# heng-hw/SpaCap3D

Measured on AMD Instinct MI355X. Metric: scenes/sec (40k pts, 256 proposals) fwd+bwd, higher is better.
Workload: dtype f32; 1 GPU; cfg2: synthetic ScanRefer-shaped scans, 40000 pts x (xyz+1 ch), 256 proposals, 8 scenes/GPU; full training step (SpaCapNet fwd + loss + bwd + grad all-reduce + Adam); global_batch=8, parallelism=dp1, hip_graph=True, fps_prefetch_side_stream=True, prefetch_as_graph=True, reserved_cus_forward=8, geometry_prefetch=True, deferred_weight_gradients=True, params=9290918, allreduce_bytes=35572416

## Files before the change

include/spacap_hip.h:

```cpp
#ifndef SPACAP_HIP_H
#define SPACAP_HIP_H

#include <stddef.h>
#include <stdint.h>

#ifdef __cplusplus
extern "C" {
#endif

#define SPACAP_ABI_VERSION 5

#define SPACAP_OK 0
#define SPACAP_E_INVALID (-1)
#define SPACAP_E_LAUNCH (-2)
#define SPACAP_E_NO_DEVICE (-3)

typedef void *spacap_stream_t;

int spacap_abi_version(void);
const char *spacap_last_error(void);
int spacap_device_count(void);

int spacap_opt_n_threads(int work_size);


size_t spacap_fps_workspace_bytes(int B, int N);
int spacap_fps_f32(const float *xyz, int B, int N, int m, void *workspace, int32_t *idx,
                   spacap_stream_t stream);

int spacap_gather_points_f32(const float *points, const int32_t *idx, int B, int C, int N, int m,
                             float *out, spacap_stream_t stream);
int spacap_gather_points_grad_f32(const float *grad_out, const int32_t *idx, int B, int C, int N,
                                  int m, float *grad_points, spacap_stream_t stream);


int spacap_ball_query_f32(const float *new_xyz, const float *xyz, int B, int N, int m,
                          float radius, int nsample, int32_t *idx, spacap_stream_t stream);

size_t spacap_ball_query_grid_workspace_bytes(int B, int N);
int spacap_ball_query_grid_f32(const float *new_xyz, const float *xyz, int B, int N, int m, float radius, int nsample,
                               int32_t *idx, void *workspace, size_t workspace_bytes, spacap_stream_t stream);


int spacap_group_points_f32(const float *points, const int32_t *idx, int B, int C, int N, int P,
                            int S, float *out, spacap_stream_t stream);
size_t spacap_group_points_grad_workspace_bytes(int B, int C, int N, int P, int S);
int spacap_group_points_grad_f32(const float *grad_out, const int32_t *idx, int B, int C, int N,
                                 int P, int S, float *grad_points, void *workspace,
                                 spacap_stream_t stream);


int spacap_group_max_f32(const float *x, long rows, int S, float *out, uint8_t *arg,
                         spacap_stream_t stream);
int spacap_group_max_grad_f32(const float *grad_out, const uint8_t *arg, long rows, int S,
                              float *grad_in, spacap_stream_t stream);


int spacap_three_nn_f32(const float *unknown, const float *known, int B, int n, int m,
                        float *dist2, int32_t *idx, spacap_stream_t stream);
int spacap_three_nn_weights_f32(const float *unknown, const float *known, int B, int n, int m,
                                float *weight, int32_t *idx, spacap_stream_t stream);
int spacap_gather_xyz_f32(const float *xyz, const int32_t *idx, int B, int N, int m, float *out, spacap_stream_t stream);
int spacap_three_interpolate_f32(const float *points, const int32_t *idx, const float *weight,
                                 int B, int C, int m, int n, float *out, spacap_stream_t stream);
int spacap_three_interpolate_grad_f32(const float *grad_out, const int32_t *idx,
                                      const float *weight, int B, int C, int n, int m,
                                      float *grad_points, spacap_stream_t stream);
int spacap_three_interpolate_grad_pm_f32(const float *grad_pm, const int32_t *idx, const float *weight, int B, int C,
                                         int n, int m, float *grad_points_pm, spacap_stream_t stream);
int spacap_fp_concat_fwd_f32(const float *known, int known_pm, const int32_t *idx, const float *weight, const float *skip, int B,
                             int K1, int K2, int m, int n, float *out, spacap_stream_t stream);
int spacap_fp_concat_bwd_f32(const float *g, int B, int K1, int K2, int n, float *g1, float *g2, spacap_stream_t stream);


int spacap_mha_fwd_f32(const float *q, const float *k, const float *v, long q_sb, long q_sh,
                       long q_sl, long k_sb, long k_sh, long k_sl, long v_sb, long v_sh, long v_sl,
                       const uint8_t *mask, long mask_sb, long mask_sq, const float *bias,
                       long bias_sb, long bias_sh, long bias_sq, int B, int h, int Lq, int Lk,
                       int d_k, float scale, float dropout_p, uint64_t seed, const uint64_t *seed_dev,
                       float *out, float *p_out, float *stats, spacap_stream_t stream);

size_t spacap_mha_bwd_workspace_bytes(int B, int h, int Lq);
int spacap_mha_bwd_f32(const float *q, const float *k, const float *v, long q_sb, long q_sh,
                       long q_sl, long k_sb, long k_sh, long k_sl, long v_sb, long v_sh, long v_sl,
                       const uint8_t *mask, long mask_sb, long mask_sq, const float *bias,
                       long bias_sb, long bias_sh, long bias_sq, int B, int h, int Lq, int Lk,
                       int d_k, float scale, float dropout_p, uint64_t seed, const uint64_t *seed_dev,
                       const float *stats, const float *d_out, const float *d_p, void *workspace,
                       float *dq, float *dk, float *dv, long grad_row_stride, spacap_stream_t stream);

int spacap_mha_bwd_delta_f32(const float *q, const float *k, const float *v, long q_sb, long q_sh,
                             long q_sl, long k_sb, long k_sh, long k_sl, long v_sb, long v_sh, long v_sl,
                             const uint8_t *mask, long mask_sb, long mask_sq, const float *bias,
                             long bias_sb, long bias_sh, long bias_sq, int B, int h, int Lq, int Lk,
                             int d_k, float scale, float dropout_p, uint64_t seed, const uint64_t *seed_dev,
                             const float *stats, const float *d_out, const float *delta,
                             float *dq, float *dk, float *dv, long grad_row_stride, spacap_stream_t stream);

size_t spacap_bn_workspace_bytes(int C);
int spacap_bn_set_single_launch(int enabled);
int spacap_bn_stats_f32(const float *z, int B, int C, long L, float eps, float momentum, float *running_mean,
                        float *running_var, float *stats, void *workspace, spacap_stream_t stream);
int spacap_bn_relu_train_f32(const float *z, int B, int C, long L, float eps, float momentum, float *running_mean,
                             float *running_var, const float *gamma, const float *beta, float *stats, float *out,
                             void *workspace, spacap_stream_t stream);
int spacap_bn_relu_apply_f32(const float *z, const float *stats, const float *gamma, const float *beta, int B,
                             int C, long L, float *out, spacap_stream_t stream);
int spacap_bn_relu_max_f32(const float *z, const float *stats, const float *gamma, const float *beta, int B, int C,
                           int P, int S, float *out, uint8_t *arg, spacap_stream_t stream);
int spacap_bn_relu_bwd_f32(const float *z, const float *stats, const float *gamma, const float *beta,
                           const float *dA, int B, int C, long L, float *dz, float *dgamma, float *dbeta,
                           void *workspace, spacap_stream_t stream);
int spacap_bn_relu_max_bwd_f32(const float *z, const float *stats, const float *gamma, const float *beta,
                               const float *dP, const uint8_t *arg, int B, int C, int P, int S, float *dz,
                               float *dgamma, float *dbeta, void *workspace, spacap_stream_t stream);

int spacap_relation_feature_fwd_f32(const float *P, const float *V, long v_sb, long v_sh, long v_sl, int B,
                                    int H, int K, int D, float *R, spacap_stream_t stream);
int spacap_relation_feature_bwd_f32(const float *dR, const float *P, const float *V, long v_sb, long v_sh,
                                    long v_sl, int B, int H, int K, int D, float *dP, float *dV,
                                    spacap_stream_t stream);

int spacap_relation_l1_fwd_f32(const float *P, const float *U, const float *b1, int B, int H, int K, int C,
                               float *H1, spacap_stream_t stream);
int spacap_relation_l1_isplit(void);
int spacap_relation_l1_supported(int H, int K, int C);
int spacap_relation_l1_blocks(int B, int K, int C);
int spacap_relation_l1_bwd_f32(const float *dH1, const float *H1, const float *P, const float *U, int B, int H,
                               int K, int C, float *dP, float *dU, float *db_part, spacap_stream_t stream);

int spacap_relation_fused_leave_cus(int n);
int spacap_relation_fused_supported(int H, int K, int C, int n_out);
int spacap_relation_fused_nparts(int B, int K);
int spacap_relation_fused_zsplit(int B, int K, int nparts);
int spacap_relation_fused_part_floats(void);
int spacap_relation_fused_fwd_f32(const float *P, const float *U, const float *b1, const float *W2, const float *b2,
                                  const float *W3, const float *b3, int B, int K, float *hid2, float *pred,
                                  spacap_stream_t stream);
int spacap_relation_fused_bwd_f32(const float *dpred, const float *hid2, const float *P, const float *U, const float *b1,
                                  const float *W2, const float *W3, int B, int K, int nparts, int zslots, float *dP,
                                  float *dU, float *part, spacap_stream_t stream);
int spacap_relation_fused_sel_zsplit(int B, int K, int nparts);
size_t spacap_relation_fused_sel_workspace_bytes(int B, int K);
int spacap_relation_fused_sel_lists_f32(const float *dpred, int B, int K, int zslots, float *dP, float *dU, void *workspace,
                                        spacap_stream_t stream);
int spacap_relation_fused_bwd_sel_f32(const float *dpred, const float *hid2, const float *P, const float *U, const float *b1,
                                      const float *W2, const float *W3, int B, int K, int nparts, int zslots, float *dP,
                                      float *dU, float *part, void *workspace, spacap_stream_t stream);

int spacap_caption_prep_fwd_f32(const float *xyz, const float *ref, const float *src, const float *memory,
                                const int64_t *tok, const float *emb, const float *pe, int B, int K, int D, int T, int V,
                                float p, uint64_t seed, const uint64_t *seed_dev, float *x0, uint8_t *mask, int64_t *idx,
                                float *dist, uint8_t *good, float *pred, int32_t *counter, spacap_stream_t stream);
int spacap_caption_prep_bwd_f32(const float *g, const int64_t *tok, const int64_t *idx, int B, int K, int D, int T, int V,
                                float p, uint64_t seed, const uint64_t *seed_dev, float *d_rows, float *d_emb,
                                spacap_stream_t stream);
int spacap_caption_prep_rows_fwd_f32(const float *src, const float *memory, const int64_t *prop, const int64_t *tok,
                                     const float *emb, const float *pe, int B, int K, int M, int S, int D, int T, int V, float p,
                                     uint64_t seed, const uint64_t *seed_dev, float *x0, uint8_t *mask, spacap_stream_t stream);
int spacap_caption_prep_rows_bwd_f32(const float *g, const int64_t *tok, const int64_t *prop, int B, int K, int M, int S, int D,
                                     int T, int V, float p, uint64_t seed, const uint64_t *seed_dev, float *d_rows, float *d_emb,
                                     spacap_stream_t stream);


int spacap_layernorm_fwd_f32(const float *x, const float *a, const float *b, long rows, int D, float eps,
                             float *y, float *stats, spacap_stream_t stream);
size_t spacap_layernorm_bwd_workspace_bytes(long rows, int D);
int spacap_layernorm_bwd_f32(const float *x, const float *a, const float *stats, const float *dy, long rows,
                             int D, float eps, float *dx, float *da, float *db, void *workspace,
                             spacap_stream_t stream);
int spacap_layernorm_bwd_add_f32(const float *x, const float *a, const float *stats, const float *dy, const float *addend,
                                 long rows, int D, float eps, float *dx, float *da, float *db, void *workspace,
                                 spacap_stream_t stream);

int spacap_sa_nparts(void);
int spacap_sa_wgrad_slabs(long R, int CK, int CP, int pooled);
int spacap_sa_mlp_supported(int C1, int C2, int C3);
int spacap_sa_l1_fwd_f32(const float *Y, const float *feat, const float *xyz, const float *new_xyz,
                         const int32_t *idx, const float *W1, int ldw, float rdiv, int B, int Np, int N, int S,
                         int C1, float *z1, double *part, spacap_stream_t stream);
int spacap_sa_bn_finalize_f32(const double *part, int C, long count, float eps, float momentum, const float *gamma,
                              const float *beta, float *running_mean, float *running_var, float *stats,
                              spacap_stream_t stream);
int spacap_sa_mid_fwd_f32(const float *zin, const float *st_in, const float *W, long R, int Cin, int Cout,
                          float *zout, double *part, spacap_stream_t stream);
int spacap_gemm_rows_supported(int Cin, int Cout);
int spacap_gemm_rows_f32(const float *x, const float *W, long R, int Cin, int Cout, float *out, spacap_stream_t stream);
int spacap_sa_mid_fwd_pool_supported(int Cin, int Cout, int S);
int spacap_sa_reserve_cus(int n);
int spacap_sa_mid_fwd_pool_f32(const float *zin, const float *st_in, const float *W, const float *gamma_out, long R,
                               int Cin, int Cout, int S, float *zout, double *part, float *cand_v, uint8_t *cand_i,
                               spacap_stream_t stream);
int spacap_sa_pool_finalize_f32(const float *cand_v, const uint8_t *cand_i, const float *stats, const float *gamma, long G,
                                int S, int C, float *out, uint8_t *arg, float *zmax, spacap_stream_t stream);
int spacap_sa_pool_fwd_f32(const float *z, const float *stats, long G, int S, int C, float *out, uint8_t *arg,
                           spacap_stream_t stream);
int spacap_sa_pool_bwd_f32(const float *dout, const float *out, const uint8_t *arg, const float *z, const float *zmax,
                           const float *stats, long G, int S, int C, float *dym, double *part,
                           spacap_stream_t stream);
long spacap_sa_l3bwd_part_floats(int C2, int C3);
int spacap_sa_l3bwd_dw_f32(const float *partW, int nparts, const float *coef3, const float *W3, int C3, int C2, double *sums,
                           float *dW3, spacap_stream_t stream);
int spacap_sa_wgrad_pool_supported(int C2, int C3, int S);
int spacap_sa_wgrad_pool_parts(long R, int C2, int C3, int S);
int spacap_sa_wgrad_pool_f32(const float *dym, const uint8_t *arg, int S, const float *coef3, const float *z2, const float *st2,
                             long R, int C3, int C2, float *partW, spacap_stream_t stream);
int spacap_sa_bwd_finalize_f32(const double *part, int C, long count, const float *stats, float *coef,
                               float *dgamma, float *dbeta, spacap_stream_t stream);
int spacap_sa_dgrad_f32(const float *dy, const uint8_t *arg, int S, const float *zk, const float *coef,
                        const float *Wk, const float *zp, const float *st_p, long R, int CK, int CP, float *dyp,
                        double *part, spacap_stream_t stream);
int spacap_sa_dgrad_l1_f32(const float *dy, const float *zk, const float *coef, const float *Wk, const float *zp,
                           const float *st_p, const float *feat, const float *xyz, const float *new_xyz,
                           const int32_t *idx, float rdiv, int B, int Np, int N, int S, int CK, int CP, double *part,
                           float *part_l1, spacap_stream_t stream);
int spacap_sa_l1_dw_f32(const float *part_l1, int nparts, const float *coef, int C1, int ldw, float *dW1, spacap_stream_t stream);

int spacap_sa_l1_stats_f32(const float *feat, const float *xyz, const float *new_xyz, const int32_t *idx, const float *W1,
                           int ldw, float rdiv, int B, int Np, int N, int S, int C1, float *rel4, double *part,
                           spacap_stream_t stream);
int spacap_sa_l1_moments_f32(const float *feat, const float *xyz, const float *new_xyz, const int32_t *idx, float rdiv, int B, int Np,
                             int N, int S, float *rel4, double *mom, spacap_stream_t stream);
int spacap_sa_l1_moments_finalize_f32(const double *mom, const float *W1, int ldw, int has_feat, int C1, long count, float eps,
                                      float momentum, const float *gamma, const float *beta, float *running_mean, float *running_var,
                                      float *stats, spacap_stream_t stream);
int spacap_sa_mid_fwd_l1in_f32(const float *rel4, const float *W1, int ldw, int has_feat, const float *st_in, const float *W,
                               long R, float *zout, double *part, spacap_stream_t stream);
int spacap_sa_wgrad_l1in_f32(const float *dy, const float *zk, const float *coef, const float *rel4, const float *W1, int ldw,
                             int has_feat, const float *st_p, long R, float *partW, spacap_stream_t stream);
int spacap_sa_dgrad_l1in_f32(const float *dy, const float *zk, const float *coef, const float *Wk, const float *rel4,
                             const float *W1, int ldw, int has_feat, const float *st_p, int B, int N, int S, double *part,
                             float *part_l1, spacap_stream_t stream);
int spacap_sa_dgrad_wgrad_l1in_slabs(long R);
int spacap_sa_dgrad_wgrad_l1in_f32(const float *dy, const float *zk, const float *coef, const float *Wk, const float *rel4,
                                   const float *W1, int ldw, int has_feat, const float *st_p, int B, int N, int S, double *part,
                                   float *part_l1, float *partW, spacap_stream_t stream);
int spacap_sa_wgrad_f32(const float *dy, const uint8_t *arg, int S, const float *zk, const float *coef,
                        const float *zp, const float *st_p, long R, int CK, int CP, float *partW,
                        spacap_stream_t stream);
int spacap_sa_l1_bwd_f32(float *dy1, const float *z1, const float *coef, const float *feat, const float *xyz,
                         const float *new_xyz, const int32_t *idx, const float *W1, int ldw, float rdiv, int B,
                         int Np, int N, int S, int C1, float *partW, float *drel, int write_dz,
                         spacap_stream_t stream);
size_t spacap_sa_rows_scatter_workspace_bytes(int B, int Np, long E);
int spacap_sa_rows_scatter_f32(const float *dz, const int32_t *idx, int B, int Np, long E, int C, float *out,
                               void *workspace, spacap_stream_t stream);
int spacap_sa_rows_index_f32(const int32_t *idx, int B, int Np, long E, void *workspace, spacap_stream_t stream);
int spacap_sa_rows_gather_f32(const float *dz, int B, int Np, long E, int C, const void *workspace, float *out,
                              spacap_stream_t stream);
int spacap_sa_drel_sums_f32(const float *drel, int B, int Np, int N, int S, const void *workspace, float *dxyz, float *dnew,
                            spacap_stream_t stream);
int spacap_sa_dw1_assemble_f32(const float *pw1, int n1, const float *pf, int nf, int C1, int Cf, float *dW1, spacap_stream_t stream);

int spacap_linear_wgrad_slabs(long R, int CK, int CP);
int spacap_linear_wgrad_f32(const float *g, const float *x, long R, int CK, int CP, int with_bias, float *part,
                            spacap_stream_t stream);
int spacap_linear_wgrad_nslab_f32(const float *g, const float *x, long R, int CK, int CP, int with_bias, int nslab, float *part,
                                  spacap_stream_t stream);
int spacap_linear_wgrad_slabs_batched(long R, int CK, int CP);
int spacap_linear_wgrad_batched_f32(const float *const *g, const float *const *x, const long *R, const int *CK,
                                    const int *CP, const int *with_bias, const int *nslabs, float *const *part, int njobs,
                                    spacap_stream_t stream);

int spacap_relu_dropout_fwd_f32(const float *x, long n, float p, uint64_t seed, const uint64_t *seed_dev,
                                float *out, spacap_stream_t stream);
int spacap_relu_dropout_bwd_f32(const float *g, const float *y, long n, float p, float *dx, spacap_stream_t stream);
int spacap_dropout_add_fwd_f32(const float *res, const float *y, long n, float p, uint64_t seed,
                               const uint64_t *seed_dev, float *out, spacap_stream_t stream);
int spacap_dropout_add_bwd_f32(const float *g, long n, float p, uint64_t seed, const uint64_t *seed_dev,
                               float *out, spacap_stream_t stream);

int spacap_scene_aug_doubles(void);
int spacap_scene_sample_augment_f32(const float *const *scene_feat, const int32_t *const *scene_ins,
                                    const uint8_t *const *scene_isobj, const float *const *scene_color,
                                    const int32_t *choices, const double *aug, int B, int P, int C, int augment,
                                    float *pc, int32_t *ins_out, uint8_t *isobj_out, float *color_out,
                                    spacap_stream_t stream);
int spacap_scene_sample_augment_map_f32(const float *const *scene_feat, const int32_t *const *scene_ins,
                                        const uint8_t *const *scene_isobj, const float *const *scene_color,
                                        const int32_t *choices, const double *aug, int B, int P, int C, int augment,
                                        int C_out, const int *dst_off, float *pc, int32_t *ins_out, uint8_t *isobj_out,
                                        float *color_out, spacap_stream_t stream);
int spacap_scene_gather_rows_f32(const float *const *src, const int32_t *choices, int B, int P, int W, float *out,
                                 int out_stride, int out_off, spacap_stream_t stream);
size_t spacap_scene_votes_workspace_bytes(int B, int max_inst);
int spacap_scene_votes_f32(const float *pc, const int32_t *ins, const uint8_t *isobj, int B, int P, int C,
                           int max_inst, void *workspace, float *votes, int64_t *vmask, spacap_stream_t stream);

int spacap_adam_flat_f32(float *p, const float *g, float *m, float *v, long n, float lr, float beta1, float beta2,
                         float eps, float weight_decay, const float *step, float grad_scale,
                         const int64_t *skip_if_nonzero, spacap_stream_t stream);

int spacap_det_npart(void);
int spacap_det_losses_fwd_f32(const float *net, const float *center, const float *agg_xyz, const float *gt_center,
                              const float *box_mask, const int64_t *heading_cls_label, const float *heading_res_label,
                              const int64_t *size_cls_label, const float *size_res_label, const int64_t *sem_cls_label,
                              const float *mean_size, const float *seed_xyz, const float *vote_xyz,
                              const int32_t *seed_inds, const float *vote_label, const int64_t *vote_mask, int B, int K,
                              int M, int NSEED, int N, int NH, int NS, int NC, float near_thr, float far_thr, float w0,
                              float w1, int64_t *obj_label, float *obj_mask, int64_t *assignment, float *dnet_num,
                              float *dcenter_num, float *dvote_num, float *part, float *losses, float *inv_den,
                              spacap_stream_t stream);
int spacap_det_losses_bwd_f32(const float *dnet_num, const float *dcenter_num, const float *dvote_num,
                              const float *grad_losses, const float *inv_den, int B, int K, int NSEED, int NH, int NS,
                              int NC, float *dnet, float *dcenter, float *dvote, spacap_stream_t stream);

long spacap_rel_loss_nparts(int B, int K);
int spacap_rel_loss_fwd_f32(const float *pred, const int64_t *assignment, const int64_t *box_mask_int,
                            const int64_t *obj_label, const int64_t *x_label, const int64_t *y_label,
                            const int64_t *z_label, int B, int K, int M, float *dnum, float *part, float *out,
                            spacap_stream_t stream);
int spacap_rel_loss_bwd_f32(const float *dnum, const float *grad_losses, const float *out, int B, int K, float *dpred,
                            spacap_stream_t stream);

int spacap_sum_slabs_f32(const float *part, int nslab, long n, float *out, spacap_stream_t stream);
int spacap_sum_slabs_batched_f32(const float *const *parts, float *const *outs, const long *n, const int *nslabs, int nseg,
                                 spacap_stream_t stream);

int spacap_linear_dgrad_mask_f32(const float *g, const float *W, const float *y, float scale, long R, int CK, int CP,
                                 float *dx, spacap_stream_t stream);

int spacap_rel_tail_fwd_f32(const float *hid1, const float *W2, const float *b2, const float *W3, const float *b3, long R,
                            float *hid2, float *pred, spacap_stream_t stream);
int spacap_rel_tail_bwd_nparts(long R);
int spacap_rel_tail_bwd_f32(const float *dpred, const float *W3, const float *hid2, long R, float *dz2, float *part,
                            spacap_stream_t stream);

int spacap_conv1x1_wgrad_slabs(int B, int CO, int CI, int N);
int spacap_conv1x1_wgrad_f32(const float *g, const float *x, int B, int CO, int CI, int N, float *part,
                             spacap_stream_t stream);
int spacap_conv1x1_wgrad_slabs_batched(int B, int CO, int CI, int N);
int spacap_conv1x1_wgrad_batched_f32(const float *const *g, const float *const *x, const int *B, const int *CO, const int *CI,
                                     const int *N, const int *nslabs, const int *with_bias, float *const *part, int njobs,
                                     spacap_stream_t stream);

int spacap_dense_rows_slices(long R, int K, int CO);
int spacap_dense_rows_f32(const float *a, long lda, long a_grp, long a_gstride, long a_skip, const float *W, long ldw, int trans_w,
                          const float *bias, long R, int K, int CO, float *out, long ldo, long o_grp, long o_gstride, long o_skip,
                          int o_zero, int slices, long slice_stride, int batch, long a_zstride, long w_zstride,
                          spacap_stream_t stream);
int spacap_dense_sum_slices_f32(const float *parts, int S, long n, long stride, float *out, spacap_stream_t stream);
int spacap_dense_wgrad_small_f32(const float *G, long ldg, const float *X, long ldx, long x_grp, long x_gstride, long x_skip, long R,
                                 int M, int N, float *dW, float *db, spacap_stream_t stream);
int spacap_dense_wgrad_blocks_slabs(long R);
int spacap_dense_wgrad_blocks_f32(const float *G, long ldg, const float *X, long ldx, long R, int Z, int M, int N, int nslab,
                                  float *part, spacap_stream_t stream);

int spacap_dense_wgrad_tall_slabs(long R, int M, int N);
int spacap_dense_wgrad_tall_f32(const float *G, long ldg, const float *X, long ldx, long R, int M, int N, int nslab, float *part,
                                spacap_stream_t stream);

int spacap_gemm_bf3_supported(int K, int N);
int spacap_gemm_bf3_split_w_f32(const float *W, long ldw, int N, int K, int trans, void *Wp, spacap_stream_t stream);
int spacap_gemm_bf3_f32(const float *A, long lda, const void *Wp, const float *bias, long R, int K, int N, int relu, float *out, long ldo,
                        spacap_stream_t stream);
int spacap_gemm_bf3_wgrad_slabs(long R, int N, int K);
int spacap_rel_wide_tail_supported(int C);
int spacap_rel_wide_tail_nparts(long R);
int spacap_rel_wide_tail_bwd_f32(const float *dpred, const float *W3, const float *hid2, long R, int C, int nparts, float *dz2, float *part,
                                 spacap_stream_t stream);
int spacap_rel_wide_l1_supported(int H, int K, int C);
int spacap_rel_wide_transpose_f32(const float *in, float *out, int B, int H, int K, int to_t, spacap_stream_t stream);
int spacap_rel_wide_l1_fwd_f32(const float *Pt, const float *U, const float *b1, int B, int H, int K, int C, float *hid1,
                               spacap_stream_t stream);
int spacap_rel_wide_l1_bwd_f32(const float *dh1, const float *hid1, const float *Pt, const float *U, int B, int H, int K, int C,
                               float *dPt, float *dU, float *db_part, spacap_stream_t stream);

int spacap_linear_rows_supported(long R, int K, int CO);
int spacap_linear_rows_f32(const float *a, const float *W, const float *bias, long R, int K, int CO, int trans_w,
                           float *out, spacap_stream_t stream);

int spacap_l2norm_rows_fwd_f32(const float *x, long rows, int D, float *y, float *inv_norm, spacap_stream_t stream);
int spacap_l2norm_rows_bwd_f32(const float *g, const float *y, const float *inv_norm, long rows, int D, float *dx,
                               spacap_stream_t stream);

int spacap_cap_loss_fwd_f32(const float *logits, const int64_t *target, const uint8_t *good, int B, int W, int V, int tstride,
                            float *logp, float *rowstat, float *out, spacap_stream_t stream);
int spacap_cap_loss_bwd_f32(const float *logp, const int64_t *target, const uint8_t *good, const float *out, const float *gloss,
                            int B, int W, int V, int tstride, float *dlogits, spacap_stream_t stream);

int spacap_proposal_decode_fwd_f32(const float *net, const float *agg_xyz, const float *mean_size, const double *mean_size_f64,
                                   int B, int K, int NH, int NS, int NC, float *nt, float *center, float *heading_res, float *size_res, double *corners,
                                   int64_t *bbox_mask, int64_t *sem_cls, int64_t *size_cls, spacap_stream_t stream);
int spacap_proposal_decode_bwd_f32(const float *g_nt, const float *g_center, const float *g_heading_res, const float *g_size_res,
                                   const float *mean_size, int B, int K, int NH, int NS, int NC, float *d_net, spacap_stream_t stream);

int spacap_loss_tail_fwd_f32(const float *det, const float *cap, const float *rel, const int64_t *obj_label, const float *obj_mask,
                             const int64_t *bbox_mask, int n, float *out, float *loss, spacap_stream_t stream);
int spacap_loss_tail_bwd_f32(const float *g_loss, float *g_det, float *g_cap, float *g_rel, spacap_stream_t stream);

typedef struct {
  int mode;
  long R;
  const float *a1;
  const float *w1;
  const float *bias1;
  int k1;
  float drop_p;
  float eps;
  uint64_t seed;
  const uint64_t *seed_dev;
  const float *res;
  float *x_out;
  const float *ln_a;
  const float *ln_b;
  float *n_out;
  float *stats;
  const float *x_ln;
  const float *g;
  float *part;
  const float *w2;
  const float *bias2;
  float *out2;
  int n2;
  int nparts;
  const float *attn_out;
  float *delta_out;
  int lq;
} spacap_tf_rows_args;
int spacap_tf_rows_f32(const spacap_tf_rows_args *args, spacap_stream_t stream);
int spacap_tf_rows_parts(long R);
int spacap_tf_ffn1_f32(const float *x, const float *W, const float *bias, long R, int N, float drop_p, uint64_t seed,
                       const uint64_t *seed_dev, float *h, spacap_stream_t stream);
int spacap_tf_ffn_f32(int mode, const float *x, const float *Wa, const float *Wb, const float *bias, const float *y, long R, int dff,
                      float drop_p, uint64_t seed, const uint64_t *seed_dev, float *hid, float *part, spacap_stream_t stream);
long spacap_tf_ffn_pieces_elems(int dff);
int spacap_tf_ffn_split_f32(const float *const *w1, const float *const *w2, void *const *pieces, int nlayers, int dff,
                            spacap_stream_t stream);
int spacap_tf_ffn_bf3_f32(int mode, const float *x, const void *pieces, const float *bias, const float *y, long R, int dff, float drop_p,
                          uint64_t seed, const uint64_t *seed_dev, float *hid, float *part, spacap_stream_t stream);
int spacap_decode_attn_f32(const float *qkv, float *kcache, float *vcache, long R, int h, int d_k, int T, int t, float scale,
                           float *out, spacap_stream_t stream);
size_t spacap_decode_word_workspace_bytes(long R, int V);
int spacap_decode_word_f32(const float *x, const void *Wp, const float *bias, long R, int V, const float *lut, float scale,
                           const float *pe_row, int64_t *ys, int ys_ld, int t_out, float *x_next, void *workspace,
                           spacap_stream_t stream);
size_t spacap_beam_topw_workspace_bytes(long rows, int V, int W);
int spacap_beam_topw_f32(const float *x, const void *Wp, const float *bias, long rows, int V, int W, float *top_logp, int32_t *top_word,
                         void *workspace, spacap_stream_t stream);
int spacap_decode_attn_beam_f32(const float *qkv, float *kcache, float *vcache, const int8_t *anc, long R, int W, int h, int d_k, int T,
                                int t, float scale, float *out, spacap_stream_t stream);
int spacap_beam_step_f32(const float *top_logp, const int32_t *top_word, long R, int W, int V, int T, int t, int eos, const float *score_in,
                         const int32_t *fin_in, const int32_t *len_in, float *score_out, int32_t *fin_out, int32_t *len_out,
                         const int8_t *anc_old, int8_t *anc_new, int8_t *trace_parent, int32_t *trace_word, const float *lut, float scale,
                         const float *pe_row, float *x_next, spacap_stream_t stream);
int spacap_beam_finish_f32(const float *score, const int32_t *len, const int8_t *trace_parent, const int32_t *trace_word, long R, int W,
                           int n_words, double alpha, int64_t *ys, float *best_score, int64_t *all_tokens, float *all_scores,
                           int32_t *all_len, spacap_stream_t stream);
size_t spacap_sample_word_workspace_bytes(long rows, int V, int top_k);
int spacap_sample_word_f32(const float *x, const void *Wp, const float *bias, long rows, int V, int top_k, float inv_tau, uint64_t seed,
                           const uint64_t *seed_dev, int n_words, int step, int eos, const float *lut, float scale, const float *pe_row,
                           int64_t *ys, float *score, int32_t *length, int32_t *finished, float *xw, void *workspace,
                           spacap_stream_t stream);
int spacap_tf_gemm_splits(long R, int K, int N);
int spacap_tf_gemm_f32(const float *a, const float *W, long R, int K, int N, int trans_w, int nsplit, float *out,
                       spacap_stream_t stream);
int spacap_tf_dgrad_mask_f32(const float *g, const float *W, const float *y, float scale, long R, int K, int N, float *out,
                             spacap_stream_t stream);

int spacap_conv1x1_cm_supported(int CI, int CO, long N);
int spacap_conv1x1_cm_f32(int mode, const float *W, const float *in, const float *bias, int B, int CI, int CO, long N,
                          float *out, spacap_stream_t stream);

int spacap_vote_assemble_fwd_f32(const float *net, const float *seed_xyz, const float *seed_feat, int B, int C, int N,
                                 float *vote_xyz, float *vote_feat, spacap_stream_t stream);
int spacap_vote_assemble_bwd_f32(const float *g_xyz, const float *g_feat, int B, int C, int N, float *d_net, float *d_seed,
                                 spacap_stream_t stream);

int spacap_copy_batched(const void *const *src, void *const *dst, const long *nbytes, int njobs, spacap_stream_t stream);

int spacap_stream_delay(int microseconds, spacap_stream_t stream);
int spacap_stream_wait_ge(const int64_t *flag, int64_t value, int timeout_ms, int64_t *err, spacap_stream_t stream);
int spacap_stream_signal(int64_t *flag, const int64_t *value, spacap_stream_t stream);

int spacap_lab_stamp(uint64_t *slot, spacap_stream_t stream);


size_t spacap_points_in_box_workspace_bytes(int B, int N, int K);
int spacap_points_in_box_f32(const float *point_clouds, int B, int N, int C, const double *bbox_corner, int K, void *workspace,
                             size_t workspace_bytes, spacap_stream_t stream);

#define SPACAP_PP_REMOVE_EMPTY 1
#define SPACAP_PP_CLS_NMS 2
#define SPACAP_PP_OLD_TYPE 4
#define SPACAP_PP_GT_F32 8

int spacap_detection_nms_f32(const float *objectness, const int64_t *sem_cls, const float *sem_cls_scores, int NC,
                             const double *bbox_corner, const void *workspace, int B, int N, int K, const double *gt_corner,
                             int M, const int64_t *object_assignment, int flags, int min_points, double nms_iou,
                             float conf_thresh, double min_iou, float *obj_prob, int32_t *count, uint8_t *nonempty,
                             uint8_t *pred_mask, float *conf, uint8_t *valid, double *iou, uint8_t *good,
                             spacap_stream_t stream);


#define SPACAP_AP_EXISTS 0x80

int spacap_detection_match_f32(const double *bbox_corner, const uint8_t *valid, const float *conf, const float *obj_prob,
                               const int64_t *sem_cls, int B, int K, int NC, const double *gt_corner,
                               const int64_t *sem_cls_label, const uint8_t *box_label_mask, int M, const double *thresholds,
                               int T, float *score, uint8_t *flags, int16_t *index, int32_t *npos, spacap_stream_t stream);

int spacap_ap_curve_f64(const uint8_t *flags, int64_t L, const int64_t *count, const int32_t *npos, int NC, int T, double *rec,
                        double *prec, double *ap, double *last_rec, spacap_stream_t stream);


int spacap_caption_select_i32(const int64_t *tokens, const int64_t *nms_mask, const uint8_t *good_bbox_mask,
                              const int64_t *dataset_idx, const int64_t *scene_object_ids, const int64_t *object_assignment,
                              int B, int K, int L, int M, const int32_t *key_table, int n_items, int n_obj, int nkeys, int sos,
                              int eos, uint64_t *stamp, uint64_t *counter, int32_t *cand_tok, int32_t *cand_len,
                              spacap_stream_t stream);

int spacap_caption_score_f64(const int32_t *cand_tok, const int32_t *cand_len, int nkeys, const int32_t *ref_tok, int64_t n_tok,
                             const int32_t *ref_off, const int32_t *ref_len, int64_t n_ref, const int32_t *key_ref_off,
                             const uint64_t *df_code, const double *df_idf, const int64_t *df_off, double log_nkeys,
                             int32_t *bleu, double *rouge, double *cider, spacap_stream_t stream);


int spacap_caption_reward_f64(const int64_t *tokens, int rows, int rows_per_scene, int L, const int64_t *dataset_idx,
                              const int64_t *object_id, const int32_t *key_table, int n_items, int n_obj, int nkeys, int sos,
                              int eos, const int32_t *ref_tok, int64_t n_tok, const int32_t *ref_off, const int32_t *ref_len,
                              int64_t n_ref, const int32_t *key_ref_off, const uint64_t *df_code, const double *df_idf,
                              const int64_t *df_off, double log_nkeys, double *cider, int32_t *key, int32_t *length,
                              int64_t *tf_tok, spacap_stream_t stream);

int spacap_scst_loss_fwd_f32(const float *logits, const int64_t *words, const int32_t *length, const double *reward,
                             const double *baseline, const uint8_t *count, int R, int S, int W, int V, float *pair, uint8_t *hit,
                             float *adv, float *rowlogp, float *out, spacap_stream_t stream);
int spacap_scst_loss_bwd_f32(const float *logits, const int64_t *words, const int32_t *length, const float *pair, const float *adv,
                             const float *out, const float *gloss, int R, int W, int V, float *dlogits, spacap_stream_t stream);

int spacap_scst_select_f32(const float *xyz, const float *center_label, const float *box_label_mask,
                           const int64_t *scene_object_ids, const int64_t *dataset_idx, const int32_t *key_table, int B, int K,
                           int G, int M, int n_items, int n_obj, int nkeys, float near2, int64_t *prop, int64_t *obj,
                           int32_t *slot_of, int32_t *key, float *dist, int32_t *n_sel, spacap_stream_t stream);


int spacap_dense_caption_select(const uint8_t *valid, const float *obj_prob, const int64_t *sem_cls, const double *bbox_corner,
                                const int64_t *tokens, int B, int K, int L, int sos, int eos, int32_t *count, int32_t *index,
                                float *score, int32_t *cls, double *corners, int32_t *out_tokens, int32_t *length,
                                spacap_stream_t stream);


size_t spacap_multiview_workspace_bytes(int F);

int spacap_multiview_map_f32(const float *points, int N, const float *depth, const float *pose, int F, int H, int W, float fx,
                             float fy, float cx, float cy, float depth_min, float depth_max, float accuracy, const float *corners,
                             void *workspace, size_t workspace_bytes, int32_t *map, spacap_stream_t stream);

int spacap_multiview_features_f32(const float *points, int N, const float *depth, const float *pose, int F, int H, int W,
                                  float fx, float fy, float cx, float cy, float depth_min, float depth_max, float accuracy,
                                  const float *corners, const float *feats, int C, int mode, void *workspace,
                                  size_t workspace_bytes, float *acc, spacap_stream_t stream);

int spacap_multiview_vote_i32(const float *points, int N, const float *depth, const float *pose, int F, int H, int W, float fx,
                              float fy, float cx, float cy, float depth_min, float depth_max, float accuracy, const float *corners,
                              const int32_t *labels, void *workspace, size_t workspace_bytes, uint32_t *state, int32_t *voted,
                              spacap_stream_t stream);


size_t spacap_enet_param_floats(void);
size_t spacap_enet_bottleneck_param_floats(int kind, int cin, int cout);

size_t spacap_enet_workspace_bytes(int B, int H, int W);

int spacap_enet_initial_f32(const float *images, int B, int H, int W, const float *params, float *out, spacap_stream_t stream);

int spacap_enet_bottleneck_f32(const float *in, int B, int h, int w, int cin, int cout, int kind, int dilation,
                               const float *params, void *workspace, size_t workspace_bytes, float *out, spacap_stream_t stream);

int spacap_enet_encode_f32(const float *images, int B, int H, int W, const float *params, size_t n_params, void *workspace,
                           size_t workspace_bytes, float *out, spacap_stream_t stream);

int spacap_enet_encode_u8(const uint8_t *images, int B, int H, int W, float mean0, float mean1, float mean2, float std0,
                          float std1, float std2, const float *params, size_t n_params, void *workspace, size_t workspace_bytes,
                          float *out, spacap_stream_t stream);


size_t spacap_scene_export_workspace_bytes(int N, int M);

int spacap_scene_normals_f32(const float *xyz, int N, const int32_t *faces, int F, void *workspace, size_t workspace_bytes,
                             float *normals, spacap_stream_t stream);

int spacap_scene_relations_f64(const double *bbox, int M, int32_t *rel, spacap_stream_t stream);

int spacap_scene_export_f32(const float *xyz, const float *rgb, int N, const int32_t *faces, int F, const int32_t *seg,
                            const int32_t *seg_ins, const int32_t *seg_sem, int S, const int32_t *box_label, int M,
                            const double *axis_align, void *workspace, size_t workspace_bytes, float *vert, float *aligned_vert,
                            int32_t *ins, int32_t *sem, double *bbox, double *aligned_bbox, int32_t *rel, spacap_stream_t stream);

#ifdef __cplusplus
}
#endif
#endif
```

spacap3d_amd/_native.py:

```python
import ctypes
import os

import torch

_HERE = os.path.dirname(os.path.abspath(__file__))
LIB_PATH = os.path.join(_HERE, "lib", "libspacap_hip.so")
ABI_VERSION = 5

_i = ctypes.c_int
_l = ctypes.c_long
_f = ctypes.c_float
_p = ctypes.c_void_p
_u64 = ctypes.c_uint64

SIGNATURES = {
    "spacap_abi_version": (_i, []),
    "spacap_last_error": (ctypes.c_char_p, []),
    "spacap_device_count": (_i, []),
    "spacap_opt_n_threads": (_i, [_i]),
    "spacap_fps_workspace_bytes": (ctypes.c_size_t, [_i, _i]),
    "spacap_fps_f32": (_i, [_p, _i, _i, _i, _p, _p, _p]),
    "spacap_gather_points_f32": (_i, [_p, _p, _i, _i, _i, _i, _p, _p]),
    "spacap_gather_points_grad_f32": (_i, [_p, _p, _i, _i, _i, _i, _p, _p]),
    "spacap_ball_query_f32": (_i, [_p, _p, _i, _i, _i, _f, _i, _p, _p]),
    "spacap_ball_query_grid_workspace_bytes": (ctypes.c_size_t, [_i, _i]),
    "spacap_ball_query_grid_f32": (_i, [_p, _p, _i, _i, _i, _f, _i, _p, _p, ctypes.c_size_t, _p]),
    "spacap_group_points_f32": (_i, [_p, _p, _i, _i, _i, _i, _i, _p, _p]),
    "spacap_group_points_grad_workspace_bytes": (ctypes.c_size_t, [_i, _i, _i, _i, _i]),
    "spacap_group_points_grad_f32": (_i, [_p, _p, _i, _i, _i, _i, _i, _p, _p, _p]),
    "spacap_group_max_f32": (_i, [_p, _l, _i, _p, _p, _p]),
    "spacap_group_max_grad_f32": (_i, [_p, _p, _l, _i, _p, _p]),
    "spacap_three_nn_f32": (_i, [_p, _p, _i, _i, _i, _p, _p, _p]),
    "spacap_three_nn_weights_f32": (_i, [_p, _p, _i, _i, _i, _p, _p, _p]),
    "spacap_gather_xyz_f32": (_i, [_p, _p, _i, _i, _i, _p, _p]),
    "spacap_three_interpolate_f32": (_i, [_p, _p, _p, _i, _i, _i, _i, _p, _p]),
    "spacap_three_interpolate_grad_f32": (_i, [_p, _p, _p, _i, _i, _i, _i, _p, _p]),
    "spacap_three_interpolate_grad_pm_f32": (_i, [_p, _p, _p, _i, _i, _i, _i, _p, _p]),
    "spacap_bn_workspace_bytes": (ctypes.c_size_t, [_i]),
    "spacap_bn_set_single_launch": (_i, [_i]),
    "spacap_bn_stats_f32": (_i, [_p, _i, _i, _l, _f, _f, _p, _p, _p, _p, _p]),
    "spacap_bn_relu_apply_f32": (_i, [_p, _p, _p, _p, _i, _i, _l, _p, _p]),
    "spacap_bn_relu_train_f32": (_i, [_p, _i, _i, _l, _f, _f, _p, _p, _p, _p, _p, _p, _p, _p]),
    "spacap_bn_relu_max_f32": (_i, [_p, _p, _p, _p, _i, _i, _i, _i, _p, _p, _p]),
    "spacap_bn_relu_bwd_f32": (_i, [_p, _p, _p, _p, _p, _i, _i, _l, _p, _p, _p, _p, _p]),
    "spacap_bn_relu_max_bwd_f32": (_i, [_p, _p, _p, _p, _p, _p, _i, _i, _i, _i, _p, _p, _p, _p, _p]),
    "spacap_relation_feature_fwd_f32": (_i, [_p, _p, _l, _l, _l, _i, _i, _i, _i, _p, _p]),
    "spacap_relation_feature_bwd_f32": (_i, [_p, _p, _p, _l, _l, _l, _i, _i, _i, _i, _p, _p, _p]),
    "spacap_relation_l1_isplit": (_i, []),
    "spacap_relation_l1_supported": (_i, [_i, _i, _i]),
    "spacap_relation_l1_blocks": (_i, [_i, _i, _i]),
    "spacap_relation_l1_fwd_f32": (_i, [_p, _p, _p, _i, _i, _i, _i, _p, _p]),
    "spacap_relation_l1_bwd_f32": (_i, [_p, _p, _p, _p, _i, _i, _i, _i, _p, _p, _p, _p]),
    "spacap_relation_fused_supported": (_i, [_i, _i, _i, _i]),
    "spacap_relation_fused_leave_cus": (_i, [_i]),
    "spacap_relation_fused_zsplit": (_i, [_i, _i, _i]),
    "spacap_relation_fused_nparts": (_i, [_i, _i]),
    "spacap_relation_fused_part_floats": (_i, []),
    "spacap_relation_fused_fwd_f32": (_i, [_p] * 7 + [_i, _i, _p, _p, _p]),
    "spacap_relation_fused_bwd_f32": (_i, [_p] * 7 + [_i, _i, _i, _i, _p, _p, _p, _p]),
    "spacap_relation_fused_sel_zsplit": (_i, [_i, _i, _i]),
    "spacap_relation_fused_sel_workspace_bytes": (ctypes.c_size_t, [_i, _i]),
    "spacap_relation_fused_sel_lists_f32": (_i, [_p, _i, _i, _i, _p, _p, _p, _p]),
    "spacap_relation_fused_bwd_sel_f32": (_i, [_p] * 7 + [_i, _i, _i, _i, _p, _p, _p, _p, _p]),
    "spacap_caption_prep_fwd_f32": (_i, [_p] * 7 + [_i] * 5 + [_f, _u64, _p] + [_p] * 7 + [_p]),
    "spacap_caption_prep_bwd_f32": (_i, [_p] * 3 + [_i] * 5 + [_f, _u64, _p, _p, _p, _p]),
    "spacap_caption_prep_rows_fwd_f32": (_i, [_p] * 6 + [_i] * 7 + [_f, _u64, _p] + [_p] * 2 + [_p]),
    "spacap_caption_prep_rows_bwd_f32": (_i, [_p] * 3 + [_i] * 7 + [_f, _u64, _p, _p, _p, _p]),
    "spacap_conv1x1_cm_supported": (_i, [_i, _i, _l]),
    "spacap_conv1x1_cm_f32": (_i, [_i, _p, _p, _p, _i, _i, _i, _l, _p, _p]),
    "spacap_sa_l1_stats_f32": (_i, [_p, _p, _p, _p, _p, _i, _f, _i, _i, _i, _i, _i, _p, _p, _p]),
    "spacap_sa_l1_moments_f32": (_i, [_p, _p, _p, _p, _f, _i, _i, _i, _i, _p, _p, _p]),
    "spacap_sa_l1_moments_finalize_f32": (_i, [_p, _p, _i, _i, _i, _l, _f, _f, _p, _p, _p, _p, _p, _p]),
    "spacap_sa_mid_fwd_l1in_f32": (_i, [_p, _p, _i, _i, _p, _p, _l, _p, _p, _p]),
    "spacap_sa_wgrad_l1in_f32": (_i, [_p, _p, _p, _p, _p, _i, _i, _p, _l, _p, _p]),
    "spacap_sa_dgrad_l1in_f32": (_i, [_p, _p, _p, _p, _p, _p, _i, _i, _p, _i, _i, _i, _p, _p, _p]),
    "spacap_sa_dgrad_wgrad_l1in_slabs": (_i, [_l]),
    "spacap_sa_dgrad_wgrad_l1in_f32": (_i, [_p, _p, _p, _p, _p, _p, _i, _i, _p, _i, _i, _i, _p, _p, _p, _p]),
    "spacap_sa_l1_dw_f32": (_i, [_p, _i, _p, _i, _i, _p, _p]),
    "spacap_vote_assemble_fwd_f32": (_i, [_p, _p, _p, _i, _i, _i, _p, _p, _p]),
    "spacap_vote_assemble_bwd_f32": (_i, [_p, _p, _i, _i, _i, _p, _p, _p]),
    "spacap_copy_batched": (_i, [_p, _p, _p, _i, _p]),
    "spacap_lab_stamp": (_i, [_p, _p]),
    "spacap_points_in_box_workspace_bytes": (ctypes.c_size_t, [_i, _i, _i]),
    "spacap_points_in_box_f32": (_i, [_p, _i, _i, _i, _p, _i, _p, ctypes.c_size_t, _p]),
    "spacap_detection_nms_f32": (_i, [_p, _p, _p, _i, _p, _p, _i, _i, _i, _p, _i, _p, _i, _i, ctypes.c_double, _f,
                                      ctypes.c_double] + [_p] * 8 + [_p]),
    "spacap_detection_match_f32": (_i, [_p] * 5 + [_i, _i, _i] + [_p] * 3 + [_i, _p, _i] + [_p] * 4 + [_p]),
    "spacap_ap_curve_f64": (_i, [_p, ctypes.c_int64, _p, _p, _i, _i] + [_p] * 4 + [_p]),
    "spacap_caption_select_i32": (_i, [_p] * 6 + [_i] * 4 + [_p] + [_i] * 5 + [_p] * 4 + [_p]),
    "spacap_caption_score_f64": (_i, [_p, _p, _i, _p, ctypes.c_int64, _p, _p, ctypes.c_int64, _p, _p, _p, _p,
                                      ctypes.c_double, _p, _p, _p, _p]),
    "spacap_caption_reward_f64": (_i, [_p, _i, _i, _i, _p, _p, _p, _i, _i, _i, _i, _i, _p, ctypes.c_int64, _p, _p, ctypes.c_int64,
                                       _p, _p, _p, _p, ctypes.c_double, _p, _p, _p, _p, _p]),
    "spacap_scst_loss_fwd_f32": (_i, [_p] * 6 + [_i] * 4 + [_p] * 5 + [_p]),
    "spacap_scst_loss_bwd_f32": (_i, [_p] * 7 + [_i] * 3 + [_p, _p]),
    "spacap_scst_select_f32": (_i, [_p] * 6 + [_i] * 7 + [_f] + [_p] * 6 + [_p]),
    "spacap_dense_caption_select": (_i, [_p] * 5 + [_i] * 5 + [_p] * 7 + [_p]),
    "spacap_multiview_workspace_bytes": (ctypes.c_size_t, [_i]),
    "spacap_multiview_map_f32": (_i, [_p, _i, _p, _p, _i, _i, _i] + [_f] * 7 + [_p, _p, ctypes.c_size_t, _p, _p]),
    "spacap_multiview_features_f32": (_i, [_p, _i, _p, _p, _i, _i, _i] + [_f] * 7 + [_p, _p, _i, _i, _p, ctypes.c_size_t, _p, _p]),
    "spacap_multiview_vote_i32": (_i, [_p, _i, _p, _p, _i, _i, _i] + [_f] * 7 + [_p, _p, _p, ctypes.c_size_t, _p, _p, _p]),
    "spacap_scene_export_workspace_bytes": (ctypes.c_size_t, [_i, _i]),
    "spacap_scene_normals_f32": (_i, [_p, _i, _p, _i, _p, ctypes.c_size_t, _p, _p]),
    "spacap_scene_relations_f64": (_i, [_p, _i, _p, _p]),
    "spacap_scene_export_f32": (_i, [_p, _p, _i, _p, _i, _p, _p, _p, _i, _p, _i, _p, _p, ctypes.c_size_t] + [_p] * 8),
    "spacap_enet_param_floats": (ctypes.c_size_t, []),
    "spacap_enet_bottleneck_param_floats": (ctypes.c_size_t, [_i, _i, _i]),
    "spacap_enet_workspace_bytes": (ctypes.c_size_t, [_i, _i, _i]),
    "spacap_enet_initial_f32": (_i, [_p, _i, _i, _i, _p, _p, _p]),
    "spacap_enet_bottleneck_f32": (_i, [_p, _i, _i, _i, _i, _i, _i, _i, _p, _p, ctypes.c_size_t, _p, _p]),
    "spacap_enet_encode_f32": (_i, [_p, _i, _i, _i, _p, ctypes.c_size_t, _p, ctypes.c_size_t, _p, _p]),
    "spacap_enet_encode_u8": (_i, [_p, _i, _i, _i] + [_f] * 6 + [_p, ctypes.c_size_t, _p, ctypes.c_size_t, _p, _p]),
    "spacap_stream_delay": (_i, [_i, _p]),
    "spacap_stream_wait_ge": (_i, [_p, _l, _i, _p, _p]),
    "spacap_stream_signal": (_i, [_p, _p, _p]),
    "spacap_sa_nparts": (_i, []),
    "spacap_sa_wgrad_slabs": (_i, [_l, _i, _i, _i]),
    "spacap_sa_mlp_supported": (_i, [_i, _i, _i]),
    "spacap_sa_l1_fwd_f32": (_i, [_p, _p, _p, _p, _p, _p, _i, _f, _i, _i, _i, _i, _i, _p, _p, _p]),
    "spacap_sa_bn_finalize_f32": (_i, [_p, _i, _l, _f, _f, _p, _p, _p, _p, _p, _p]),
    "spacap_sa_mid_fwd_f32": (_i, [_p, _p, _p, _l, _i, _i, _p, _p, _p]),
    "spacap_sa_pool_fwd_f32": (_i, [_p, _p, _l, _i, _i, _p, _p, _p]),
    "spacap_gemm_rows_supported": (_i, [_i, _i]),
    "spacap_gemm_rows_f32": (_i, [_p, _p, _l, _i, _i, _p, _p]),
    "spacap_sa_mid_fwd_pool_supported": (_i, [_i, _i, _i]),
    "spacap_sa_reserve_cus": (_i, [_i]),
    "spacap_sa_mid_fwd_pool_f32": (_i, [_p, _p, _p, _p, _l, _i, _i, _i, _p, _p, _p, _p, _p]),
    "spacap_sa_pool_finalize_f32": (_i, [_p, _p, _p, _p, _l, _i, _i, _p, _p, _p, _p]),
    "spacap_sa_pool_bwd_f32": (_i, [_p, _p, _p, _p, _p, _p, _l, _i, _i, _p, _p, _p]),
    "spacap_fp_concat_fwd_f32": (_i, [_p, _i, _p, _p, _p, _i, _i, _i, _i, _i, _p, _p]),
    "spacap_fp_concat_bwd_f32": (_i, [_p, _i, _i, _i, _i, _p, _p, _p]),
    "spacap_dense_rows_slices": (_i, [_l, _i, _i]),
    "spacap_dense_rows_f32": (_i, [_p, _l, _l, _l, _l, _p, _l, _i, _p, _l, _i, _i, _p, _l, _l, _l, _l, _i, _i, _l, _i, _l, _l, _p]),
    "spacap_dense_sum_slices_f32": (_i, [_p, _i, _l, _l, _p, _p]),
    "spacap_dense_wgrad_small_f32": (_i, [_p, _l, _p, _l, _l, _l, _l, _l, _i, _i, _p, _p, _p]),
    "spacap_dense_wgrad_blocks_slabs": (_i, [_l]),
    "spacap_dense_wgrad_blocks_f32": (_i, [_p, _l, _p, _l, _l, _i, _i, _i, _i, _p, _p]),
    "spacap_dense_wgrad_tall_slabs": (_i, [_l, _i, _i]),
    "spacap_dense_wgrad_tall_f32": (_i, [_p, _l, _p, _l, _l, _i, _i, _i, _p, _p]),
    "spacap_gemm_bf3_supported": (_i, [_i, _i]),
    "spacap_gemm_bf3_split_w_f32": (_i, [_p, _l, _i, _i, _i, _p, _p]),
    "spacap_gemm_bf3_f32": (_i, [_p, _l, _p, _p, _l, _i, _i, _i, _p, _l, _p]),
    "spacap_gemm_bf3_wgrad_slabs": (_i, [_l, _i, _i]),
    "spacap_rel_wide_tail_supported": (_i, [_i]),
    "spacap_rel_wide_tail_nparts": (_i, [_l]),
    "spacap_rel_wide_tail_bwd_f32": (_i, [_p, _p, _p, _l, _i, _i, _p, _p, _p]),
    "spacap_rel_wide_l1_supported": (_i, [_i, _i, _i]),
    "spacap_rel_wide_transpose_f32": (_i, [_p, _p, _i, _i, _i, _i, _p]),
    "spacap_rel_wide_l1_fwd_f32": (_i, [_p, _p, _p, _i, _i, _i, _i, _p, _p]),
    "spacap_rel_wide_l1_bwd_f32": (_i, [_p, _p, _p, _p, _i, _i, _i, _i, _p, _p, _p, _p]),
    "spacap_sa_l3bwd_part_floats": (_l, [_i, _i]),
    "spacap_sa_l3bwd_dw_f32": (_i, [_p, _i, _p, _p, _i, _i, _p, _p, _p]),
    "spacap_sa_wgrad_pool_supported": (_i, [_i, _i, _i]),
    "spacap_sa_wgrad_pool_parts": (_i, [_l, _i, _i, _i]),
    "spacap_sa_wgrad_pool_f32": (_i, [_p, _p, _i, _p, _p, _p, _l, _i, _i, _p, _p]),
    "spacap_sa_bwd_finalize_f32": (_i, [_p, _i, _l, _p, _p, _p, _p, _p]),
    "spacap_sa_dgrad_f32": (_i, [_p, _p, _i, _p, _p, _p, _p, _p, _l, _i, _i, _p, _p, _p]),
    "spacap_sa_dgrad_l1_f32": (_i, [_p] * 10 + [_f] + [_i] * 6 + [_p, _p, _p]),
    "spacap_sa_wgrad_f32": (_i, [_p, _p, _i, _p, _p, _p, _p, _l, _i, _i, _p, _p]),
    "spacap_sa_l1_bwd_f32": (_i, [_p, _p, _p, _p, _p, _p, _p, _p, _i, _f, _i, _i, _i, _i, _i, _p, _p, _i, _p]),
    "spacap_sa_rows_scatter_workspace_bytes": (ctypes.c_size_t, [_i, _i, _l]),
    "spacap_sa_rows_scatter_f32": (_i, [_p, _p, _i, _i, _l, _i, _p, _p, _p]),
    "spacap_sa_rows_index_f32": (_i, [_p, _i, _i, _l, _p, _p]),
    "spacap_sa_rows_gather_f32": (_i, [_p, _i, _i, _l, _i, _p, _p, _p]),
    "spacap_sa_drel_sums_f32": (_i, [_p, _i, _i, _i, _i, _p, _p, _p, _p]),
    "spacap_sa_dw1_assemble_f32": (_i, [_p, _i, _p, _i, _i, _i, _p, _p]),
    "spacap_relu_dropout_fwd_f32": (_i, [_p, _l, _f, _u64, _p, _p, _p]),
    "spacap_relu_dropout_bwd_f32": (_i, [_p, _p, _l, _f, _p, _p]),
    "spacap_dropout_add_fwd_f32": (_i, [_p, _p, _l, _f, _u64, _p, _p, _p]),
    "spacap_dropout_add_bwd_f32": (_i, [_p, _l, _f, _u64, _p, _p, _p]),
    "spacap_scene_aug_doubles": (_i, []),
    "spacap_scene_sample_augment_f32": (_i, [_p, _p, _p, _p, _p, _p, _i, _i, _i, _i, _p, _p, _p, _p, _p]),
    "spacap_scene_sample_augment_map_f32": (_i, [_p, _p, _p, _p, _p, _p, _i, _i, _i, _i, _i, _p, _p, _p, _p, _p, _p]),
    "spacap_scene_gather_rows_f32": (_i, [_p, _p, _i, _i, _i, _p, _i, _i, _p]),
    "spacap_l2norm_rows_fwd_f32": (_i, [_p, _l, _i, _p, _p, _p]),
    "spacap_l2norm_rows_bwd_f32": (_i, [_p, _p, _p, _l, _i, _p, _p]),
    "spacap_cap_loss_fwd_f32": (_i, [_p, _p, _p, _i, _i, _i, _i, _p, _p, _p, _p]),
    "spacap_cap_loss_bwd_f32": (_i, [_p, _p, _p, _p, _p, _i, _i, _i, _i, _p, _p]),
    "spacap_scene_votes_workspace_bytes": (ctypes.c_size_t, [_i, _i]),
    "spacap_scene_votes_f32": (_i, [_p, _p, _p, _i, _i, _i, _i, _p, _p, _p, _p]),
    "spacap_det_npart": (_i, []),
    "spacap_det_losses_fwd_f32": (_i, [_p] * 16 + [_i] * 8 + [_f] * 4 + [_p] * 9 + [_p]),
    "spacap_det_losses_bwd_f32": (_i, [_p] * 5 + [_i] * 6 + [_p] * 3 + [_p]),
    "spacap_rel_loss_nparts": (_l, [_i, _i]),
    "spacap_rel_loss_fwd_f32": (_i, [_p] * 7 + [_i] * 3 + [_p] * 3 + [_p]),
    "spacap_rel_loss_bwd_f32": (_i, [_p] * 3 + [_i] * 2 + [_p, _p]),
    "spacap_sum_slabs_f32": (_i, [_p, _i, _l, _p, _p]),
    "spacap_sum_slabs_batched_f32": (_i, [_p, _p, _p, _p, _i, _p]),
    "spacap_adam_flat_f32": (_i, [_p, _p, _p, _p, _l, _f, _f, _f, _f, _f, _p, _f, _p, _p]),
    "spacap_linear_dgrad_mask_f32": (_i, [_p, _p, _p, _f, _l, _i, _i, _p, _p]),
    "spacap_rel_tail_fwd_f32": (_i, [_p, _p, _p, _p, _p, _l, _p, _p, _p]),
    "spacap_rel_tail_bwd_nparts": (_i, [_l]),
    "spacap_rel_tail_bwd_f32": (_i, [_p, _p, _p, _l, _p, _p, _p]),
    "spacap_conv1x1_wgrad_slabs": (_i, [_i, _i, _i, _i]),
    "spacap_conv1x1_wgrad_f32": (_i, [_p, _p, _i, _i, _i, _i, _p, _p]),
    "spacap_conv1x1_wgrad_slabs_batched": (_i, [_i, _i, _i, _i]),
    "spacap_conv1x1_wgrad_batched_f32": (_i, [_p, _p, _p, _p, _p, _p, _p, _p, _p, _i, _p]),
    "spacap_linear_rows_supported": (_i, [_l, _i, _i]),
    "spacap_linear_rows_f32": (_i, [_p, _p, _p, _l, _i, _i, _i, _p, _p]),
    "spacap_linear_wgrad_slabs": (_i, [_l, _i, _i]),
    "spacap_linear_wgrad_f32": (_i, [_p, _p, _l, _i, _i, _i, _p, _p]),
    "spacap_linear_wgrad_nslab_f32": (_i, [_p, _p, _l, _i, _i, _i, _i, _p, _p]),
    "spacap_linear_wgrad_slabs_batched": (_i, [_l, _i, _i]),
    "spacap_linear_wgrad_batched_f32": (_i, [_p, _p, _p, _p, _p, _p, _p, _p, _i, _p]),
    "spacap_layernorm_fwd_f32": (_i, [_p, _p, _p, _l, _i, _f, _p, _p, _p]),
    "spacap_layernorm_bwd_workspace_bytes": (ctypes.c_size_t, [_l, _i]),
    "spacap_layernorm_bwd_f32": (_i, [_p, _p, _p, _p, _l, _i, _f, _p, _p, _p, _p, _p]),
    "spacap_layernorm_bwd_add_f32": (_i, [_p, _p, _p, _p, _p, _l, _i, _f, _p, _p, _p, _p, _p]),
    "spacap_proposal_decode_fwd_f32": (_i, [_p, _p, _p, _p, _i, _i, _i, _i, _i, _p, _p, _p, _p, _p, _p, _p, _p, _p]),
    "spacap_proposal_decode_bwd_f32": (_i, [_p, _p, _p, _p, _p, _i, _i, _i, _i, _i, _p, _p]),
    "spacap_loss_tail_fwd_f32": (_i, [_p, _p, _p, _p, _p, _p, _i, _p, _p, _p]),
    "spacap_loss_tail_bwd_f32": (_i, [_p, _p, _p, _p, _p]),
    "spacap_tf_rows_f32": (_i, [_p, _p]),
    "spacap_tf_rows_parts": (_i, [_l]),
    "spacap_tf_ffn1_f32": (_i, [_p, _p, _p, _l, _i, _f, _u64, _p, _p, _p]),
    "spacap_tf_ffn_f32": (_i, [_i, _p, _p, _p, _p, _p, _l, _i, _f, _u64, _p, _p, _p, _p]),
    "spacap_tf_ffn_pieces_elems": (_l, [_i]),
    "spacap_tf_ffn_split_f32": (_i, [_p, _p, _p, _i, _i, _p]),
    "spacap_tf_ffn_bf3_f32": (_i, [_i, _p, _p, _p, _p, _l, _i, _f, _u64, _p, _p, _p, _p]),
    "spacap_decode_attn_f32": (_i, [_p, _p, _p, _l, _i, _i, _i, _i, _f, _p, _p]),
    "spacap_decode_word_workspace_bytes": (ctypes.c_size_t, [_l, _i]),
    "spacap_decode_word_f32": (_i, [_p, _p, _p, _l, _i, _p, _f, _p, _p, _i, _i, _p, _p, _p]),
    "spacap_beam_topw_workspace_bytes": (ctypes.c_size_t, [_l, _i, _i]),
    "spacap_beam_topw_f32": (_i, [_p, _p, _p, _l, _i, _i, _p, _p, _p, _p]),
    "spacap_decode_attn_beam_f32": (_i, [_p, _p, _p, _p, _l, _i, _i, _i, _i, _i, _f, _p, _p]),
    "spacap_beam_step_f32": (_i, [_p, _p, _l, _i, _i, _i, _i, _i] + [_p] * 6 + [_p] * 4 + [_p, _f, _p, _p, _p]),
    "spacap_beam_finish_f32": (_i, [_p, _p, _p, _p, _l, _i, _i, ctypes.c_double, _p, _p, _p, _p, _p, _p]),
    "spacap_sample_word_workspace_bytes": (ctypes.c_size_t, [_l, _i, _i]),
    "spacap_sample_word_f32": (_i, [_p, _p, _p, _l, _i, _i, _f, _u64, _p, _i, _i, _i, _p, _f, _p, _p, _p, _p, _p, _p, _p, _p]),
    "spacap_tf_gemm_splits": (_i, [_l, _i, _i]),
    "spacap_tf_gemm_f32": (_i, [_p, _p, _l, _i, _i, _i, _i, _p, _p]),
    "spacap_tf_dgrad_mask_f32": (_i, [_p, _p, _p, _f, _l, _i, _i, _p, _p]),
    "spacap_mha_fwd_f32": (_i, [_p, _p, _p] + [_l] * 9 + [_p, _l, _l, _p, _l, _l, _l]
                           + [_i] * 5 + [_f, _f, _u64, _p, _p, _p, _p, _p]),
    "spacap_mha_bwd_workspace_bytes": (ctypes.c_size_t, [_i, _i, _i]),
    "spacap_mha_bwd_delta_f32": (_i, [_p, _p, _p] + [_l] * 9 + [_p, _l, _l, _p, _l, _l, _l]
                                 + [_i] * 5 + [_f, _f, _u64, _p, _p, _p, _p, _p, _p, _p, _l, _p]),
    "spacap_mha_bwd_f32": (_i, [_p, _p, _p] + [_l] * 9 + [_p, _l, _l, _p, _l, _l, _l]
                           + [_i] * 5 + [_f, _f, _u64, _p, _p, _p, _p, _p, _p, _p, _p, _l, _p]),
}


class TfRowsArgs(ctypes.Structure):
    _fields_ = [("mode", _i), ("R", _l), ("a1", _p), ("w1", _p), ("bias1", _p), ("k1", _i), ("drop_p", _f), ("eps", _f),
                ("seed", _u64), ("seed_dev", _p), ("res", _p), ("x_out", _p), ("ln_a", _p), ("ln_b", _p), ("n_out", _p),
                ("stats", _p), ("x_ln", _p), ("g", _p), ("part", _p), ("w2", _p), ("bias2", _p), ("out2", _p), ("n2", _i), ("nparts", _i), ("attn_out", _p), ("delta_out", _p), ("lq", _i)]


def _load():
    if not os.path.exists(LIB_PATH):
        raise ImportError(
            f"{LIB_PATH} not found: the HIP extension is not built. Run "
            "`python -c 'import __graft_entry__ as g; g.build()'` (or `make -C spacap3d_amd/csrc`). "
            "spacap3d_amd has no CPU or PyTorch fallback for its native operators.")
    lib = ctypes.CDLL(LIB_PATH)
    for name, (res, args) in SIGNATURES.items():
        fn = getattr(lib, name)
        fn.restype = res
        fn.argtypes = args
    got = lib.spacap_abi_version()
    if got != ABI_VERSION:
        raise ImportError(f"libspacap_hip.so ABI {got} != expected {ABI_VERSION}: rebuild the extension")
    return lib


lib = _load()


def check(rc: int, what: str) -> None:
    if rc != 0:
        msg = lib.spacap_last_error().decode("utf-8", "replace")
        raise RuntimeError(f"{what} failed (code {rc}): {msg}")


_DEFERRED = None


class deferred_slab_sums:

    def __enter__(self):
        global _DEFERRED
        self._prev = _DEFERRED
        self.items = []
        self.jobs = []
        self.conv_jobs = []
        _DEFERRED = self
        return self

    def __exit__(self, *exc):
        global _DEFERRED
        _DEFERRED = self._prev
        if exc[0] is None:
            self.flush()
        return False

    def has_job_for(self, part):
        ptr = part.data_ptr()
        return any(j[3].data_ptr() == ptr for j in self.jobs) or any(j[3].data_ptr() == ptr for j in self.conv_jobs)

    def outputs(self):
        return [o for _, o in self.items]

    def flush(self):
        self.run_jobs()
        self.run_sums()

    def run_jobs(self):
        import torch
        jobs, self.jobs = self.jobs, []
        if jobs:
            by_dev = {}
            for j in jobs:
                by_dev.setdefault(j[0].device, []).append(j)
            for dev, group in by_dev.items():
                k = len(group)
                arr = lambda ct, vals: (ct * k)(*vals)
                with torch.cuda.device(dev):
                    check(lib.spacap_linear_wgrad_batched_f32(
                        arr(ctypes.c_void_p, [j[0].data_ptr() for j in group]), arr(ctypes.c_void_p, [j[1].data_ptr() for j in group]),
                        arr(ctypes.c_long, [j[0].shape[0] for j in group]), arr(ctypes.c_int, [j[0].shape[1] for j in group]),
                        arr(ctypes.c_int, [j[1].shape[1] for j in group]), arr(ctypes.c_int, [int(j[2]) for j in group]),
                        arr(ctypes.c_int, [j[3].shape[0] for j in group]),
                        arr(ctypes.c_void_p, [j[3].data_ptr() for j in group]), k, torch.cuda.current_stream(dev).cuda_stream),
                        "spacap_linear_wgrad_batched_f32")
        cjobs, self.conv_jobs = self.conv_jobs, []
        if cjobs:
            by_dev = {}
            for j in cjobs:
                by_dev.setdefault(j[0].device, []).append(j)
            for dev, group in by_dev.items():
                k = len(group)
                arr = lambda ct, vals: (ct * k)(*vals)
                with torch.cuda.device(dev):
                    check(lib.spacap_conv1x1_wgrad_batched_f32(
                        arr(ctypes.c_void_p, [j[0].data_ptr() for j in group]), arr(ctypes.c_void_p, [j[1].data_ptr() for j in group]),
                        arr(ctypes.c_int, [j[2][0] for j in group]), arr(ctypes.c_int, [j[2][1] for j in group]),
                        arr(ctypes.c_int, [j[2][2] for j in group]), arr(ctypes.c_int, [j[2][3] for j in group]),
                        arr(ctypes.c_int, [j[3].shape[0] for j in group]), arr(ctypes.c_int, [int(j[4]) for j in group]),
                        arr(ctypes.c_void_p, [j[3].data_ptr() for j in group]),
                        k, torch.cuda.current_stream(dev).cuda_stream), "spacap_conv1x1_wgrad_batched_f32")

    def run_sums(self):
        import torch
        items, self.items = self.items, []
        by_dev = {}
        for part, out in items:
            by_dev.setdefault(part.device, []).append((part, out))
        for dev, group in by_dev.items():
            k = len(group)
            parts = (ctypes.c_void_p * k)(*[p.data_ptr() for p, _ in group])
            outs = (ctypes.c_void_p * k)(*[o.data_ptr() for _, o in group])
            ns = (ctypes.c_long * k)(*[o.numel() for _, o in group])
            nsl = (ctypes.c_int * k)(*[p.shape[0] for p, _ in group])
            with torch.cuda.device(dev):
                check(lib.spacap_sum_slabs_batched_f32(parts, outs, ns, nsl, k, torch.cuda.current_stream(dev).cuda_stream),
                      "spacap_sum_slabs_batched_f32")


GRAD_SLOTS = {}


class grad_slots:
    def __init__(self, table):
        self.table = table or {}

    def __enter__(self):
        global GRAD_SLOTS
        self._prev, GRAD_SLOTS = GRAD_SLOTS, self.table
        return self

    def __exit__(self, *exc):
        global GRAD_SLOTS
        GRAD_SLOTS = self._prev
        return False


def grad_slot(weight, numel):
    t = GRAD_SLOTS.get(weight.data_ptr())
    return t if (t is not None and t.numel() == numel and t.device == weight.device) else None


def sum_slabs(part, deferrable=False, out=None):
    import torch
    n = part[0].numel()
    if out is not None and (out.numel() != n or out.data_ptr() % 16 or not out.is_contiguous()):
        out = None
    if part.shape[0] == 1:
        if out is not None and not (_DEFERRED is not None and _DEFERRED.has_job_for(part)):
            out.copy_(part[0].reshape(-1))
            return out.view(part.shape[1:])
        return part[0]
    can_defer = deferrable and _DEFERRED is not None and part.is_cuda and part.data_ptr() % 16 == 0 and n % 4 == 0 \
        and part.dtype == torch.float32 and part.is_contiguous()
    if not can_defer and _DEFERRED is not None and part.is_cuda and _DEFERRED.has_job_for(part):
        _DEFERRED.run_jobs()
    if not part.is_cuda or n % 4 or part.dtype != torch.float32 or not part.is_contiguous():
        return part.sum(0)
    if can_defer:
        if out is None:
            with torch.cuda.device(part.device):
                out = torch.empty(part.shape[1:], dtype=torch.float32, device=part.device)
        else:
            out = out.view(part.shape[1:])
        _DEFERRED.items.append((part, out))
        return out
    with torch.cuda.device(part.device):
        out = torch.empty(part.shape[1:], dtype=torch.float32, device=part.device) if out is None else out.view(part.shape[1:])
        check(lib.spacap_sum_slabs_f32(part.data_ptr(), part.shape[0], n, out.data_ptr(),
                                       torch.cuda.current_stream(part.device).cuda_stream), "spacap_sum_slabs_f32")
    return out


def linear_wgrad_partials(g2, x2, with_bias, deferrable=False):
    import torch
    R, CK = g2.shape
    CP = x2.shape[1]
    nslab = int(lib.spacap_linear_wgrad_slabs(R, CK, CP))
    if nslab == 0:
        return None
    with torch.cuda.device(g2.device):
        if deferrable and _DEFERRED is not None:
            nb = int(lib.spacap_linear_wgrad_slabs_batched(R, CK, CP))
            part = torch.empty(nb, CK * CP + (CK if with_bias else 0), dtype=torch.float32, device=g2.device)
            _DEFERRED.jobs.append((g2, x2, bool(with_bias), part))
            return part
        part = torch.empty(nslab, CK * CP + (CK if with_bias else 0), dtype=torch.float32, device=g2.device)
        check(lib.spacap_linear_wgrad_f32(g2.data_ptr(), x2.data_ptr(), R, CK, CP, 1 if with_bias else 0, part.data_ptr(),
                                          torch.cuda.current_stream(g2.device).cuda_stream), "spacap_linear_wgrad_f32")
    return part


def conv1x1_wgrad_partials(g, x, B, CO, CI, N, deferrable=False, with_bias=False):
    import torch
    with torch.cuda.device(g.device):
        if deferrable and _DEFERRED is not None:
            nb = int(lib.spacap_conv1x1_wgrad_slabs_batched(B, CO, CI, N))
            part = torch.empty(nb, CO * CI + (((CO + 3) // 4) * 4 if with_bias else 0), dtype=torch.float32, device=g.device)
            _DEFERRED.conv_jobs.append((g, x, (B, CO, CI, N), part, bool(with_bias)))
            return part
        nslab = int(lib.spacap_conv1x1_wgrad_slabs(B, CO, CI, N))
        part = torch.empty(nslab, CO * CI, dtype=torch.float32, device=g.device)
        check(lib.spacap_conv1x1_wgrad_f32(g.data_ptr(), x.data_ptr(), B, CO, CI, N, part.data_ptr(),
                                           torch.cuda.current_stream(g.device).cuda_stream), "spacap_conv1x1_wgrad_f32")
    return part


def copy_batched(dsts, srcs):
    import torch
    ok = len(dsts) == len(srcs) and len(dsts) > 0 and all(
        d.is_cuda and s.is_cuda and d.device == s.device and d.dtype == s.dtype and d.shape == s.shape and d.is_contiguous()
        and s.is_contiguous() for d, s in zip(dsts, srcs))
    if not ok:
        if dsts:
            torch._foreach_copy_(list(dsts), list(srcs), non_blocking=True)
        return
    n = len(dsts)
    PA, LA = ctypes.c_void_p * n, ctypes.c_long * n
    src = PA(*[s.data_ptr() for s in srcs])
    dst = PA(*[d.data_ptr() for d in dsts])
    nb = LA(*[d.numel() * d.element_size() for d in dsts])
    dev = dsts[0].device
    with torch.cuda.device(dev):
        check(lib.spacap_copy_batched(src, dst, nb, n, torch.cuda.current_stream(dev).cuda_stream), "spacap_copy_batched")
```

spacap3d_amd/csrc/relation_fused.hip:

```cpp
#include <stdlib.h>
#include <atomic>

#include "common.hpp"
#include "launch.hpp"
#include "mfma.hpp"

namespace {

using namespace spacap::mfma;

constexpr int H = 8, C = 128, NO = 9, LDT = C + 8, TI = 8, TJ = 8, TR = TI * TJ;
constexpr int DPL = 12;
constexpr int LDB = C + 8, IMG = TR * LDB;
constexpr int LDR = TR + 8, IMGT = C * LDR;
constexpr int PART = C * C + NO * C + C + C + 16;

__device__ __forceinline__ f32x4 relu4(f32x4 v) { return f32x4{fmaxf(v[0], 0.f), fmaxf(v[1], 0.f), fmaxf(v[2], 0.f), fmaxf(v[3], 0.f)}; }

__device__ __forceinline__ size_t pair_row(int b, int K, int i0, int j0, int rr) { return ((size_t)b * K + i0 + (rr & 7)) * K + j0 + (rr >> 3); }

__device__ __forceinline__ void st_pieces(__bf16 *dst, int piece_stride, f32x4 v) {
  bf16x4 p0, p1, p2;
  split4(v, p0, p1, p2);
  *reinterpret_cast<bf16x4 *>(dst) = p0;
  *reinterpret_cast<bf16x4 *>(dst + piece_stride) = p1;
  *reinterpret_cast<bf16x4 *>(dst + 2 * piece_stride) = p2;
}
__device__ __forceinline__ void ld_pieces(const __bf16 *src, int piece_stride, bf16x8 *p) {
#pragma unroll
  for (int q = 0; q < 3; ++q) p[q] = *reinterpret_cast<const bf16x8 *>(src + q * piece_stride);
}

__device__ __forceinline__ void p_tile_request(const float *__restrict__ P, int b, int K, int i0, int j0, float *pp) {
#pragma unroll
  for (int e = 0; e < 2; ++e) {
    const int idx = threadIdx.x + 256 * e, h = idx >> 6, ii = (idx >> 3) & 7, jj = idx & 7;
    pp[e] = P[(((size_t)b * H + h) * K + i0 + ii) * K + j0 + jj];
  }
}
__device__ __forceinline__ void p_tile_request_at(const float *__restrict__ P, int b, int K, int qrow, int kcol, float *pp) {
#pragma unroll
  for (int e = 0; e < 2; ++e) {
    const int h = (threadIdx.x + 256 * e) >> 6;
    pp[e] = P[(((size_t)b * H + h) * K + qrow) * K + kcol];
  }
}
__device__ __forceinline__ void p_tile_store(const float *pp, float *s_p) {
#pragma unroll
  for (int e = 0; e < 2; ++e) {
    const int idx = threadIdx.x + 256 * e, h = idx >> 6, ii = (idx >> 3) & 7, jj = idx & 7;
    s_p[h * TR + jj * TI + ii] = pp[e];
  }
}

template <bool TRANSPOSED>
__device__ __forceinline__ void hid1_rows(const float (*uA)[4], const float *bA, const float *s_p, int w, int l15, int lg, __bf16 *img) {
  const float p0 = s_p[lg * TR + 16 * w + l15], p1 = s_p[(4 + lg) * TR + 16 * w + l15];
  const bool hi = l15 >> 3;
  const float pB[4] = {hi ? 0.f : p0, hi ? 0.f : p1, hi ? p0 : 0.f, hi ? p1 : 0.f};
  const float one = lg == 0 ? 1.f : 0.f;
#pragma unroll
  for (int n = 0; n < 8; ++n) {
    f32x4 acc = {0.f, 0.f, 0.f, 0.f};
    if (TRANSPOSED) {
      acc = MFMA16(one, bA[n], acc);
#pragma unroll
      for (int ks = 0; ks < 4; ++ks) acc = MFMA16(pB[ks], uA[n][ks], acc);
      st_pieces(img + (16 * n + l15) * LDR + 16 * w + 4 * lg, IMGT, relu4(acc));
    } else {
      acc = MFMA16(bA[n], one, acc);
#pragma unroll
      for (int ks = 0; ks < 4; ++ks) acc = MFMA16(uA[n][ks], pB[ks], acc);
      st_pieces(img + (16 * w + l15) * LDB + 16 * n + 4 * lg, IMG, relu4(acc));
    }
  }
}

__global__ __launch_bounds__(256) void rel_fused_fwd_kernel(const float *__restrict__ P, const float *__restrict__ Um,
                                                            const float *__restrict__ b1, const float *__restrict__ W2,
                                                            const float *__restrict__ b2, const float *__restrict__ W3,
                                                            const float *__restrict__ b3, int B, int K, float *__restrict__ hid2,
                                                            float *__restrict__ pred) {
  extern __shared__ __attribute__((aligned(16))) unsigned char smem_raw[];
  __bf16 *s_a = reinterpret_cast<__bf16 *>(smem_raw);
  float *s_pr = reinterpret_cast<float *>(smem_raw + 3 * IMG * 2);
  float *s_p = s_pr + 4 * TR * DPL;
  const int tid = threadIdx.x, lane = tid & 63, w = tid >> 6, l15 = lane & 15, lg = lane >> 4;
  const int NI = K / TI, NJ = K / TJ;
  const long U = (long)B * NJ * NI, u_beg = (long)blockIdx.x * U / gridDim.x, u_end = ((long)blockIdx.x + 1) * U / gridDim.x;
  bf16x8 wA[2][4][3];
  float w3r[2][4];
  f32x4 bb[2];
#pragma unroll
  for (int t = 0; t < 2; ++t) {
    const float *wp = W2 + (size_t)(32 * w + 16 * t + l15) * C + 8 * lg;
#pragma unroll
    for (int kc = 0; kc < 4; ++kc) split8(ld4(wp + 32 * kc), ld4(wp + 32 * kc + 4), wA[t][kc]);
#pragma unroll
    for (int uu = 0; uu < 4; ++uu) w3r[t][uu] = l15 < NO ? W3[l15 * C + 32 * w + 16 * t + 4 * lg + uu] : 0.f;
    bb[t] = ld4(b2 + 32 * w + 16 * t + 4 * lg);
  }
  float pp[2];
  for (long u = u_beg; u < u_end;) {
    const int grp = (int)(u / NI), ib0 = (int)(u - (long)grp * NI), ibe = (int)min((long)NI, ib0 + (u_end - u));
    const int b = grp / NJ, j0 = (grp - b * NJ) * TJ, ibeg = ib0 * TI, iend = ibe * TI;
    u += ibe - ib0;
    float uA[8][4], bA[8];
#pragma unroll
    for (int n = 0; n < 8; ++n) {
#pragma unroll
      for (int ks = 0; ks < 4; ++ks) uA[n][ks] = Um[(((size_t)b * K + j0 + 2 * w + (ks >> 1)) * H + 4 * (ks & 1) + lg) * C + 16 * n + l15];
      bA[n] = lg == 0 ? b1[16 * n + l15] : 0.f;
    }
    p_tile_request(P, b, K, ibeg, j0, pp);
    auto pred_out = [&](int i0) {
#pragma unroll
      for (int e = 0; e < 3; ++e) {
        const int idx = tid + 256 * e, ii = idx / (TJ * NO), off = idx - ii * (TJ * NO), j = off / NO, o = off - j * NO;
        if (idx < TR * NO) {
          const float *q = s_pr + (j * TI + ii) * DPL + o;
          pred[(((size_t)b * K + i0 + ii) * K + j0) * NO + off] = ((q[0] + q[TR * DPL]) + (q[2 * TR * DPL] + q[3 * TR * DPL])) + b3[o];
        }
      }
    };

    for (int i0 = ibeg; i0 < iend; i0 += TI) {
      __syncthreads();
      p_tile_store(pp, s_p);
      if (i0 > ibeg) pred_out(i0 - TI);
      if (i0 + TI < iend) p_tile_request(P, b, K, i0 + TI, j0, pp);
      __syncthreads();
      hid1_rows<false>(uA, bA, s_p, w, l15, lg, s_a);
      __syncthreads();
#pragma unroll 2
      for (int mt = 0; mt < TR / 16; ++mt) {
        f32x4 acc[2] = {{0.f, 0.f, 0.f, 0.f}, {0.f, 0.f, 0.f, 0.f}};
#pragma unroll
        for (int kc = 0; kc < 4; ++kc) {
          bf16x8 a[3];
          ld_pieces(s_a + (mt * 16 + l15) * LDB + 32 * kc + 8 * lg, IMG, a);
          acc[0] = mfma6(wA[0][kc], a, acc[0]);
          acc[1] = mfma6(wA[1][kc], a, acc[1]);
        }
        const int rr = mt * 16 + l15;
        float *hrow = hid2 + pair_row(b, K, i0, j0, rr) * C + 32 * w + 4 * lg;
        f32x4 a3 = {0.f, 0.f, 0.f, 0.f}, a3b = {0.f, 0.f, 0.f, 0.f};
#pragma unroll
        for (int t = 0; t < 2; ++t) {
          const f32x4 h = relu4(acc[t] + bb[t]);
          st4(hrow + 16 * t, h);
          a3 = MFMA16(w3r[t][0], h[0], a3);
          a3b = MFMA16(w3r[t][1], h[1], a3b);
          a3 = MFMA16(w3r[t][2], h[2], a3);
          a3b = MFMA16(w3r[t][3], h[3], a3b);
        }
        if (lg < 3) st4(&s_pr[(w * TR + rr) * DPL + 4 * lg], a3 + a3b);
      }
    }
    __syncthreads();
    pred_out(iend - TI);
  }
}

__host__ __device__ inline size_t sel_cnt_off(int, int) { return 0; }
__host__ __device__ inline size_t sel_qi_off(int B, int) { return (size_t)4 * B; }
__host__ __device__ inline size_t sel_kj_off(int B, int K) { return (size_t)4 * B + (size_t)B * K; }
__host__ __device__ inline size_t sel_rowflag_off(int B, int K) { return (size_t)4 * B + (size_t)2 * B * K; }
__host__ __device__ inline size_t sel_colflag_off(int B, int K) { return (size_t)4 * B + (size_t)3 * B * K; }
__host__ __device__ inline size_t sel_colbits_off(int B, int K) { return (size_t)4 * B + (size_t)4 * B * K; }
__host__ __device__ inline int sel_nw(int K) { return (K + 63) >> 6; }
__host__ __device__ inline size_t sel_blk_off(int B, int K) { return sel_colbits_off(B, K) + (size_t)2 * B * K * sel_nw(K); }
__host__ __device__ inline int sel_blk_stride(int K) { return 2 + 2 * (K / 8); }
__device__ __forceinline__ int clampi(int v, int hi) { return min(max(v, 0), hi); }

template <bool SEL>
__device__ __forceinline__ void rel_bwd_body(const float *__restrict__ dpred, const float *__restrict__ hid2,
                                             const float *__restrict__ P, const float *__restrict__ U,
                                             const float *__restrict__ b1, const float *__restrict__ W2,
                                             const float *__restrict__ W3, int B, int K, int Z, const int *__restrict__ ws,
                                             float *__restrict__ dP, float *__restrict__ dU, float *__restrict__ part) {
  extern __shared__ __attribute__((aligned(16))) unsigned char smem_raw[];
  __bf16 *s_h1T = reinterpret_cast<__bf16 *>(smem_raw);
  __bf16 *s_zT = s_h1T + 3 * IMGT;
  __bf16 *s_z = s_zT;
  float *s_x = reinterpret_cast<float *>(smem_raw + 2 * 3 * IMGT * 2);
  float *s_p = s_x + TR * LDT, *s_dp = s_p + H * TR;
  const int tid = threadIdx.x, lane = tid & 63, w = tid >> 6, l15 = lane & 15, lg = lane >> 4;
  const int jj = tid >> 5, c4 = tid & 31;
  const int NI = K / TI, NJ = K / TJ;
  long NU = (long)B * NJ * NI, u_beg = (long)blockIdx.x * NU / gridDim.x, u_end = ((long)blockIdx.x + 1) * NU / gridDim.x;
  long L = 0;
  bool dense = true;
  const int *cnt = SEL ? ws + sel_cnt_off(B, K) : nullptr, *blk = SEL ? ws + sel_blk_off(B, K) : nullptr;
  const int BS = sel_blk_stride(K);
  if (SEL) {
    long long nu = 0, tb = 0;
    int nim = 0;
    for (int s = tid; s < B; s += 256) {
      const int ni = clampi(cnt[4 * s + 2], NI), nj = clampi(cnt[4 * s + 3], NJ);
      nu += (long long)ni * nj;
      nim = max(nim, ni);
      tb += (long long)clampi(blk[(size_t)s * BS], NI) * clampi(blk[(size_t)s * BS + 1], NJ);
    }
#pragma unroll
    for (int m = 32; m >= 1; m >>= 1) {
      nu += __shfl_xor(nu, m);
      tb += __shfl_xor(tb, m);
      nim = max(nim, __shfl_xor(nim, m));
    }
    long long *s_nu = reinterpret_cast<long long *>(s_x);
    int *s_ni = reinterpret_cast<int *>(s_nu + 8);
    if (lane == 0) s_nu[w] = nu, s_nu[4 + w] = tb, s_ni[w] = nim;
    __syncthreads();
    nu = (s_nu[0] + s_nu[1]) + (s_nu[2] + s_nu[3]);
    tb = (s_nu[4] + s_nu[5]) + (s_nu[6] + s_nu[7]);
    nim = max(max(s_ni[0], s_ni[1]), max(s_ni[2], s_ni[3]));
    dense = tb <= nu || tb * 16 <= NU;
    if (!dense) {
      NU = nu;
      L = max((NU + gridDim.x - 1) / gridDim.x, (long)(nim + max(Z - 1, 1) - 1) / max(Z - 1, 1));
      u_beg = min(NU, (long)blockIdx.x * L);
      u_end = min(NU, ((long)blockIdx.x + 1) * L);
    }
    if (u_beg >= u_end) {
      float *po = part + (size_t)blockIdx.x * PART;
      for (int idx = tid; idx < PART; idx += 256) po[idx] = 0.f;
      return;
    }
  }
  float bA[8], w3A[8][3];
#pragma unroll
  for (int n = 0; n < 8; ++n) {
    bA[n] = lg == 0 ? b1[16 * n + l15] : 0.f;
#pragma unroll
    for (int ks = 0; ks < 3; ++ks) w3A[n][ks] = 4 * ks + lg < NO ? W3[(4 * ks + lg) * C + 16 * n + l15] : 0.f;
  }
  bf16x8 wA[2][4][3];
#pragma unroll
  for (int t = 0; t < 2; ++t)
#pragma unroll
    for (int kc = 0; kc < 4; ++kc) {
      const float *wp = W2 + (size_t)(32 * kc + 8 * lg) * C + 32 * w + 16 * t + l15;
      split8(f32x4{wp[0], wp[C], wp[2 * C], wp[3 * C]}, f32x4{wp[4 * C], wp[5 * C], wp[6 * C], wp[7 * C]}, wA[t][kc]);
    }
  const bf16x8 ones = {(__bf16)1.f, (__bf16)1.f, (__bf16)1.f, (__bf16)1.f, (__bf16)1.f, (__bf16)1.f, (__bf16)1.f, (__bf16)1.f};
  f32x4 gw[2][8], gb2[2], g3[2], d1[2], gb3 = {0.f, 0.f, 0.f, 0.f};
#pragma unroll
  for (int t = 0; t < 2; ++t) {
    gb2[t] = g3[t] = d1[t] = f32x4{0.f, 0.f, 0.f, 0.f};
#pragma unroll
    for (int n = 0; n < 8; ++n) gw[t][n] = f32x4{0.f, 0.f, 0.f, 0.f};
  }
  for (int idx = tid; idx < TR * DPL; idx += 256) s_dp[idx] = 0.f;

  f32x4 hp[TI];
  float pp[2], dq[3];
  int sc = 0, NIs = SEL ? clampi(cnt[2], NI) : NI, NJs = SEL ? clampi(cnt[3], NJ) : NJ;
  long sbeg = 0;
  for (long u = u_beg; u < u_end;) {
  int b, j0, ib0, ibe;
  long kstart;
  if (SEL && !dense) {
    while (sc + 1 < B && u >= sbeg + (long)NIs * NJs) {
      sbeg += (long)NIs * NJs;
      ++sc;
      NIs = clampi(cnt[4 * sc + 2], NI), NJs = clampi(cnt[4 * sc + 3], NJ);
    }
    const long v = u - sbeg;
    const int jb = (int)(v / NIs);
    ib0 = (int)(v - (long)jb * NIs), ibe = (int)min((long)NIs, ib0 + (u_end - u));
    b = sc, j0 = jb * TJ, kstart = sbeg + (long)jb * NIs;
  } else {
    const int grp = (int)(u / NI);
    ib0 = (int)(u - (long)grp * NI), ibe = (int)min((long)NI, ib0 + (u_end - u));
    b = grp / NJ, j0 = (grp - b * NJ) * TJ, kstart = (long)grp * NI;
  }
  u += ibe - ib0;
  const int *rfl = SEL ? blk + (size_t)b * BS + 2 : nullptr;
  auto next_tile = [&](int ib) -> int {
    if (SEL && dense)
      while (ib < ibe && !rfl[ib]) ++ib;
    return ib;
  };
  if (SEL && dense && !rfl[NI + (j0 >> 3)]) continue;
  int ib = next_tile(ib0);
  if (ib >= ibe) continue;
  int ibn = next_tile(ib + 1), ibn2 = ibn < ibe ? next_tile(ibn + 1) : ibe;
  const int *ql = SEL ? ws + sel_qi_off(B, K) + (size_t)b * K : nullptr, *kl = SEL ? ws + sel_kj_off(B, K) + (size_t)b * K : nullptr;
  auto KJ = [&](int x) -> int { return SEL && !dense ? clampi(kl[j0 + x], K - 1) : j0 + x; };
  const int kP = KJ(tid & 7), kH = KJ(jj), kU[2] = {KJ(2 * w), KJ(2 * w + 1)}, kR = KJ(2 * w + (l15 >> 3)), kZ = KJ(2 * w + (lg >> 1));
  int kD[3], iD[3], oD[3];
#pragma unroll
  for (int e = 0; e < 3; ++e) {
    const int idx = tid + 256 * e, ii = idx / (TJ * NO), off = idx - ii * (TJ * NO), j = off / NO;
    iD[e] = ii, oD[e] = off - j * NO, kD[e] = idx < TR * NO ? KJ(j) : 0;
  }
  float uA[8][4];
  f32x4 uP[8], du[8];
#pragma unroll
  for (int n = 0; n < 8; ++n) {
#pragma unroll
    for (int ks = 0; ks < 4; ++ks) uA[n][ks] = U[(((size_t)b * K + kU[ks >> 1]) * H + 4 * (ks & 1) + lg) * C + 16 * n + l15];
    uP[n] = ld4(U + (((size_t)b * K + kR) * H + (l15 & 7)) * C + 16 * n + 4 * lg);
    du[n] = f32x4{0.f, 0.f, 0.f, 0.f};
  }
  int ha = 0, hb = 0;
  auto rows_of = [&](int i0) -> int { return !SEL ? 0 : dense ? i0 + (lane & 7) : clampi(ql[i0 + (lane & 7)], K - 1); };
  auto row = [&](int i0, int h, int x) -> int { return SEL ? __shfl(h, x & 7) : i0 + x; };
  auto request = [&](int i0, int h) {
    p_tile_request_at(P, b, K, row(i0, h, (tid >> 3) & 7), kP, pp);
    int rD[3];
#pragma unroll
    for (int e = 0; e < 3; ++e) rD[e] = row(i0, h, iD[e]);
#pragma unroll
    for (int e = 0; e < 3; ++e)
      dq[e] = tid + 256 * e < TR * NO ? dpred[(((size_t)b * K + rD[e]) * K + kD[e]) * NO + oD[e]] : 0.f;
#pragma unroll
    for (int ii = 0; ii < TI; ++ii) {
      const int r = SEL ? __builtin_amdgcn_readlane(h, ii) : i0 + ii;
      hp[ii] = ld4(hid2 + (((size_t)b * K + r) * K + kH) * C + 4 * c4);
    }
  };
  ha = rows_of(ib * TI);
  if (ibn < ibe) hb = rows_of(ibn * TI);
  request(ib * TI, ha);

  for (; ib < ibe; ib = ibn, ibn = ibn2, ibn2 = ibn < ibe ? next_tile(ibn + 1) : ibe) {
    const int i0 = ib * TI;
    __syncthreads();
    const int qR = row(i0, ha, l15 & 7);
    p_tile_store(pp, s_p);
#pragma unroll
    for (int e = 0; e < 3; ++e) {
      const int idx = tid + 256 * e, ii = idx / (TJ * NO), off = idx - ii * (TJ * NO), j = off / NO, o = off - j * NO;
      if (idx < TR * NO) s_dp[(j * TI + ii) * DPL + o] = dq[e];
    }
#pragma unroll
    for (int ii = 0; ii < TI; ++ii) st4(&s_x[(jj * TI + ii) * LDT + 4 * c4], hp[ii]);
    if (ibn < ibe) {
      ha = hb;
      request(ibn * TI, ha);
      if (ibn2 < ibe) hb = rows_of(ibn2 * TI);
    }
    __syncthreads();
    float dB[3];
#pragma unroll
    for (int ks = 0; ks < 3; ++ks) dB[ks] = s_dp[(16 * w + l15) * DPL + 4 * ks + lg];
    hid1_rows<true>(uA, bA, s_p, w, l15, lg, s_h1T);
    {
#pragma unroll
      for (int n = 0; n < 8; ++n) {
        f32x4 acc = {0.f, 0.f, 0.f, 0.f};
#pragma unroll
        for (int ks = 0; ks < 3; ++ks) acc = MFMA16(dB[ks], w3A[n][ks], acc);
        const float *hx = s_x + (16 * w + 4 * lg) * LDT + 16 * n + l15;
#pragma unroll
        for (int uu = 0; uu < 4; ++uu) acc[uu] = hx[uu * LDT] > 0.f ? acc[uu] : 0.f;
        st_pieces(s_zT + (16 * n + l15) * LDR + 16 * w + 4 * lg, IMGT, acc);
      }
#pragma unroll 4
      for (int ks = 0; ks < TR / 4; ++ks) {
        const float a = l15 < NO ? s_dp[(4 * ks + lg) * DPL + l15] : 0.f;
        const float *hr = s_x + (4 * ks + lg) * LDT + 32 * w + l15;
        g3[0] = MFMA16(a, hr[0], g3[0]);
        g3[1] = MFMA16(a, hr[16], g3[1]);
        if (w == 0) gb3 = MFMA16(a, 1.f, gb3);
      }
    }
    __syncthreads();
#pragma unroll 1
    for (int kc = 0; kc < TR / 32; ++kc) {
      bf16x8 za[2][3];
      ld_pieces(s_zT + (32 * w + l15) * LDR + 32 * kc + 8 * lg, IMGT, za[0]);
      ld_pieces(s_zT + (32 * w + 16 + l15) * LDR + 32 * kc + 8 * lg, IMGT, za[1]);
#pragma unroll
      for (int n = 0; n < 8; ++n) {
        bf16x8 hb[3];
        ld_pieces(s_h1T + (16 * n + l15) * LDR + 32 * kc + 8 * lg, IMGT, hb);
        gw[0][n] = mfma6(za[0], hb, gw[0][n]);
        gw[1][n] = mfma6(za[1], hb, gw[1][n]);
      }
#pragma unroll
      for (int t = 0; t < 2; ++t)
#pragma unroll
        for (int q = 2; q >= 0; --q) gb2[t] = MFMA_B(za[t][q], ones, gb2[t]);
    }
    __syncthreads();
    {
#pragma unroll
      for (int n = 0; n < 8; ++n) {
        f32x4 acc = {0.f, 0.f, 0.f, 0.f};
#pragma unroll
        for (int ks = 0; ks < 3; ++ks) acc = MFMA16(w3A[n][ks], dB[ks], acc);
        const f32x4 h2 = ld4(&s_x[(16 * w + l15) * LDT + 16 * n + 4 * lg]);
#pragma unroll
        for (int uu = 0; uu < 4; ++uu) acc[uu] = h2[uu] > 0.f ? acc[uu] : 0.f;
        st_pieces(s_z + (16 * w + l15) * LDB + 16 * n + 4 * lg, IMG, acc);
      }
    }
    __syncthreads();
#pragma unroll 1
    for (int mt = 0; mt < TR / 16; ++mt) {
      f32x4 acc[2] = {{0.f, 0.f, 0.f, 0.f}, {0.f, 0.f, 0.f, 0.f}};
#pragma unroll
      for (int kc = 0; kc < 4; ++kc) {
        bf16x8 z[3];
        ld_pieces(s_z + (mt * 16 + l15) * LDB + 32 * kc + 8 * lg, IMG, z);
        acc[0] = mfma6(wA[0][kc], z, acc[0]);
        acc[1] = mfma6(wA[1][kc], z, acc[1]);
      }
      const int rr = mt * 16 + l15;
#pragma unroll
      for (int t = 0; t < 2; ++t) {
        const unsigned short *hb = reinterpret_cast<const unsigned short *>(s_h1T) + (32 * w + 16 * t + 4 * lg) * LDR + rr;
#pragma unroll
        for (int uu = 0; uu < 4; ++uu) acc[t][uu] = (hb[uu * LDR] & 0x7fff) ? acc[t][uu] : 0.f;
        d1[t] += acc[t];
        st4(&s_x[rr * LDT + 32 * w + 16 * t + 4 * lg], acc[t]);
      }
    }
    __syncthreads();
    {
      f32x4 acc = {0.f, 0.f, 0.f, 0.f}, accb = {0.f, 0.f, 0.f, 0.f};
#pragma unroll
      for (int q = 0; q < 8; ++q) {
        const f32x4 a = ld4(&s_x[(16 * w + l15) * LDT + 16 * q + 4 * lg]);
        acc = MFMA16(uP[q][0], a[0], acc);
        accb = MFMA16(uP[q][1], a[1], accb);
        acc = MFMA16(uP[q][2], a[2], acc);
        accb = MFMA16(uP[q][3], a[3], accb);
      }
      acc += accb;
      if ((lg >> 1) == (l15 >> 3)) {
        float *o = dP + (((size_t)b * H + 4 * (lg & 1)) * K + qR) * K + kR;
#pragma unroll
        for (int uu = 0; uu < 4; ++uu) o[(size_t)uu * K * K] = acc[uu];
      }
      const float q0 = s_p[(l15 & 7) * TR + 16 * w + (l15 >> 3) * TI + lg], q1 = s_p[(l15 & 7) * TR + 16 * w + (l15 >> 3) * TI + 4 + lg];
      const bool hi = l15 >> 3;
      const float pA[4] = {hi ? 0.f : q0, hi ? 0.f : q1, hi ? q0 : 0.f, hi ? q1 : 0.f};
#pragma unroll
      for (int ks = 0; ks < 4; ++ks) {
        const float *zr = s_x + (16 * w + 4 * ks + lg) * LDT + l15;
#pragma unroll
        for (int n = 0; n < 8; ++n) du[n] = MFMA16(pA[ks], zr[16 * n], du[n]);
      }
    }
  }
  {
    const long first = (kstart + 1) * gridDim.x;
    const int slot = (int)(blockIdx.x - (SEL && !dense ? kstart / L : (first + NU - 1) / NU - 1));
    const size_t slab = (size_t)B * K * H * C;
    float *duo = dU + (size_t)slot * slab + (((size_t)b * K + kZ) * H + 4 * (lg & 1)) * C + l15;
    if (!SEL || slot < Z) {
#pragma unroll
      for (int n = 0; n < 8; ++n)
#pragma unroll
        for (int uu = 0; uu < 4; ++uu) duo[uu * C + 16 * n] = du[n][uu];
    }
    if (!SEL && ibe == NI)
      for (int z = slot + 1; z < Z; ++z)
#pragma unroll
        for (int n = 0; n < 8; ++n)
#pragma unroll
          for (int uu = 0; uu < 4; ++uu) duo[(size_t)(z - slot) * slab + uu * C + 16 * n] = 0.f;
  }
  }
  float *po = part + (size_t)blockIdx.x * PART;
#pragma unroll
  for (int t = 0; t < 2; ++t)
#pragma unroll
    for (int n = 0; n < 8; ++n)
#pragma unroll
      for (int uu = 0; uu < 4; ++uu) po[(size_t)(32 * w + 16 * t + 4 * lg + uu) * C + 16 * n + l15] = gw[t][n][uu];
  float *p3 = po + C * C, *pb1 = p3 + NO * C, *pb2 = pb1 + C, *pb3 = pb2 + C;
#pragma unroll
  for (int t = 0; t < 2; ++t)
#pragma unroll
    for (int uu = 0; uu < 4; ++uu) {
      if (4 * lg + uu < NO) p3[(4 * lg + uu) * C + 32 * w + 16 * t + l15] = g3[t][uu];
      if (l15 == 0) pb2[32 * w + 16 * t + 4 * lg + uu] = gb2[t][uu];
    }
  if (w == 0 && l15 == 0) st4(pb3 + 4 * lg, gb3);
  __syncthreads();
  float *s_sum = s_x;
  st4(&s_sum[l15 * C + 32 * w + 4 * lg], d1[0]);
  st4(&s_sum[l15 * C + 32 * w + 16 + 4 * lg], d1[1]);
  __syncthreads();
  if (tid < C) {
    float a = 0.f;
#pragma unroll
    for (int g = 0; g < 16; ++g) a += s_sum[g * C + tid];
    pb1[tid] = a;
  }
}

__global__ __launch_bounds__(256) void rel_fused_bwd_kernel(const float *__restrict__ dpred, const float *__restrict__ hid2,
                                                            const float *__restrict__ P, const float *__restrict__ U,
                                                            const float *__restrict__ b1, const float *__restrict__ W2,
                                                            const float *__restrict__ W3, int B, int K, int Z,
                                                            float *__restrict__ dP, float *__restrict__ dU, float *__restrict__ part) {
  rel_bwd_body<false>(dpred, hid2, P, U, b1, W2, W3, B, K, Z, nullptr, dP, dU, part);
}
__global__ __launch_bounds__(256) void rel_fused_bwd_sel_kernel(const float *__restrict__ dpred, const float *__restrict__ hid2,
                                                                const float *__restrict__ P, const float *__restrict__ U,
                                                                const float *__restrict__ b1, const float *__restrict__ W2,
                                                                const float *__restrict__ W3, int B, int K, int Z,
                                                                const int *__restrict__ ws, float *__restrict__ dP,
                                                                float *__restrict__ dU, float *__restrict__ part) {
  rel_bwd_body<true>(dpred, hid2, P, U, b1, W2, W3, B, K, Z, ws, dP, dU, part);
}

__global__ __launch_bounds__(256) void rel_sel_scan_kernel(const float *__restrict__ dpred, int B, int K, int Z, int *__restrict__ ws,
                                                           float *__restrict__ dP, float *__restrict__ dU) {
  __shared__ int s_f[256];
  const int tid = threadIdx.x, lane = tid & 63, w = tid >> 6, NW = sel_nw(K);
  const size_t row = blockIdx.x;
  const int b = (int)(row / K), i = (int)(row - (size_t)b * K);
  unsigned long long *colbits = reinterpret_cast<unsigned long long *>(ws + sel_colbits_off(B, K)) + row * NW;
  bool any = false;
  for (int c0 = 0; c0 < K; c0 += 256) {
    const int nq = min(256, K - c0) * NO / 4;
    s_f[tid] = 0;
    __syncthreads();
    const float *d = dpred + (row * K + c0) * NO;
    for (int q = tid; q < nq; q += 256) {
      const f32x4 v = ld4(d + 4 * q);
#pragma unroll
      for (int c = 0; c < 4; ++c)
        if (v[c] != 0.f) s_f[(4 * q + c) / NO] = 1, any = true;
    }
    __syncthreads();
    const unsigned long long bal = __ballot(s_f[tid] != 0);
    if (lane == 0 && (c0 >> 6) + w < NW) colbits[(c0 >> 6) + w] = bal;
    __syncthreads();
  }
  const int r = __syncthreads_or(any);
  if (tid == 0) ws[sel_rowflag_off(B, K) + row] = r != 0;
  const f32x4 zero = {0.f, 0.f, 0.f, 0.f};
  for (int h = 0; h < H; ++h) {
    float *o = dP + (((size_t)b * H + h) * K + i) * K;
    for (int q = tid; q < K / 4; q += 256) st4(o + 4 * q, zero);
  }
  for (int z = 0; z < Z; ++z) {
    float *o = dU + ((size_t)z * B * K + row) * H * C;
    for (int q = tid; q < H * C / 4; q += 256) st4(o + 4 * q, zero);
  }
}

__device__ __forceinline__ int compact_list(const int *flag, int K, int *list, int *s_wc) {
  const int tid = threadIdx.x, lane = tid & 63, w = tid >> 6;
  int n = 0;
  for (int c0 = 0; c0 < K; c0 += 256) n += __syncthreads_count(c0 + tid < K && flag[c0 + tid] != 0);
  const int pad = ((n + 7) & ~7) - n;
  int base = 0;
  for (int c0 = 0; c0 < K; c0 += 256) {
    const int j = c0 + tid;
    const bool f = j < K && flag[j] != 0;
    const unsigned long long bal = __ballot(f);
    if (lane == 0) s_wc[w] = __popcll(bal);
    __syncthreads();
    int a = base + __popcll(bal & ((1ull << lane) - 1));
    for (int ww = 0; ww < w; ++ww) a += s_wc[ww];
    if (f) list[a] = j;
    else if (j < K && j - a < pad) list[n + j - a] = j;
    base += (s_wc[0] + s_wc[1]) + (s_wc[2] + s_wc[3]);
    __syncthreads();
  }
  return n;
}

__global__ __launch_bounds__(256) void rel_sel_compact_kernel(int B, int K, int *__restrict__ ws) {
  __shared__ int s_wc[4];
  const int tid = threadIdx.x, b = blockIdx.x, NW = sel_nw(K);
  const unsigned long long *colbits = reinterpret_cast<const unsigned long long *>(ws + sel_colbits_off(B, K)) + (size_t)b * K * NW;
  int *colflag = ws + sel_colflag_off(B, K) + (size_t)b * K;
  for (int j = tid; j < K; j += 256) {
    unsigned long long acc = 0;
#pragma unroll 8
    for (int i = 0; i < K; ++i) acc |= colbits[(size_t)i * NW + (j >> 6)];
    colflag[j] = (int)((acc >> (j & 63)) & 1);
  }
  __threadfence_block();
  __syncthreads();
  const int nq = compact_list(ws + sel_rowflag_off(B, K) + (size_t)b * K, K, ws + sel_qi_off(B, K) + (size_t)b * K, s_wc);
  const int nk = compact_list(colflag, K, ws + sel_kj_off(B, K) + (size_t)b * K, s_wc);
  const int *rowflag = ws + sel_rowflag_off(B, K) + (size_t)b * K;
  int *bl = ws + sel_blk_off(B, K) + (size_t)b * sel_blk_stride(K);
  const int NB = K / 8;
  int rbn = 0, cbn = 0;
  for (int c0 = 0; c0 < NB; c0 += 256) {
    const int ib = c0 + tid;
    int rf = 0, cf = 0;
    if (ib < NB) {
#pragma unroll
      for (int k = 0; k < 8; ++k) rf |= rowflag[8 * ib + k], cf |= colflag[8 * ib + k];
      bl[2 + ib] = rf != 0, bl[2 + NB + ib] = cf != 0;
    }
    rbn += __syncthreads_count(rf != 0);
    cbn += __syncthreads_count(cf != 0);
  }
  if (tid == 0) {
    int *cnt = ws + sel_cnt_off(B, K) + 4 * b;
    cnt[0] = nq, cnt[1] = nk, cnt[2] = (nq + 7) >> 3, cnt[3] = (nk + 7) >> 3;
    bl[0] = rbn, bl[1] = cbn;
  }
}

constexpr size_t FWD_LDS = (size_t)3 * IMG * 2 + (size_t)(4 * TR * DPL + H * TR) * sizeof(float);
constexpr size_t BWD_LDS = (size_t)2 * 3 * IMGT * 2 + (size_t)(TR * LDT + H * TR + TR * DPL) * sizeof(float);

static std::atomic<int> g_rel_leave{0};
inline int grid_size(int B, int K, int per_cu) {
  const long units = (long)B * (K / TJ) * (K / TI);
  const int extra = g_rel_leave.load(std::memory_order_relaxed);
  const long g = (long)per_cu * std::max(1, spacap::device_cus() - extra - spacap::launch::fwd_cus_left_free(per_cu));
  return (int)std::min(units, g);
}
inline int du_slots(int B, int K, int G) {
  const long NI = K / TI, NU = (long)B * (K / TJ) * NI;
  int z = 1;
  for (long g = 0; g < (long)B * (K / TJ); ++g) {
    const long wf = ((g * NI + 1) * G + NU - 1) / NU - 1, wl = (((g + 1) * NI) * G + NU - 1) / NU - 1;
    z = std::max(z, (int)(wl - wf + 1));
  }
  return z;
}

}

extern "C" int spacap_relation_fused_leave_cus(int n) {
  if (n < 0 || n > spacap::device_cus() / 2) return SPACAP_E_INVALID;
  g_rel_leave.store(n, std::memory_order_relaxed);
  return SPACAP_OK;
}
extern "C" int spacap_relation_fused_supported(int H_, int K, int C_, int NO_) {
  return H_ == H && C_ == C && NO_ == NO && K >= 8 && K % 8 == 0;
}
extern "C" int spacap_relation_fused_nparts(int B, int K) { return B > 0 && K >= 8 ? grid_size(B, K, 1) : 0; }
extern "C" int spacap_relation_fused_zsplit(int B, int K, int nparts) { return B > 0 && K >= 8 && nparts > 0 ? du_slots(B, K, nparts) : 0; }
extern "C" int spacap_relation_fused_part_floats(void) { return PART; }
extern "C" int spacap_relation_fused_sel_zsplit(int B, int K, int nparts) {
  return B > 0 && K >= 8 && nparts > 0 ? std::max(3, du_slots(B, K, nparts)) : 0;
}
extern "C" size_t spacap_relation_fused_sel_workspace_bytes(int B, int K) {
  return B > 0 && K >= 8 ? (sel_blk_off(B, K) + (size_t)B * sel_blk_stride(K)) * sizeof(int) : 0;
}

extern "C" int spacap_relation_fused_fwd_f32(const float *P, const float *U, const float *b1, const float *W2, const float *b2,
                                             const float *W3, const float *b3, int B, int K, float *hid2, float *pred,
                                             spacap_stream_t stream) {
  const char *what = "spacap_relation_fused_fwd_f32";
  SPACAP_REQUIRE(B >= 0 && K >= 8 && K % 8 == 0 && B <= 65535, "%s: (B=%d, K=%d) unsupported", what, B, K);
  if (B == 0) return SPACAP_OK;
  SPACAP_REQUIRE(P && U && b1 && W2 && b2 && W3 && b3 && hid2 && pred, "%s: null pointer", what);
  static unsigned long long lds_ok = 0;
  SPACAP_CHECK_HIP(spacap::allow_dynamic_lds(reinterpret_cast<const void *>(&rel_fused_fwd_kernel), (int)FWD_LDS, lds_ok), what);
  hipLaunchKernelGGL(rel_fused_fwd_kernel, dim3(grid_size(B, K, 2)), dim3(256), FWD_LDS, spacap::as_stream(stream), P, U, b1, W2, b2, W3,
                     b3, B, K, hid2, pred);
  SPACAP_CHECK_LAUNCH(what);
  return SPACAP_OK;
}

extern "C" int spacap_relation_fused_bwd_f32(const float *dpred, const float *hid2, const float *P, const float *U, const float *b1,
                                             const float *W2, const float *W3, int B, int K, int nparts, int zslots, float *dP,
                                             float *dU, float *part, spacap_stream_t stream) {
  const char *what = "spacap_relation_fused_bwd_f32";
  SPACAP_REQUIRE(B >= 0 && K >= 8 && K % 8 == 0 && B <= 65535, "%s: (B=%d, K=%d) unsupported", what, B, K);
  if (B == 0) return SPACAP_OK;
  SPACAP_REQUIRE(dpred && hid2 && P && U && b1 && W2 && W3 && dP && dU && part, "%s: null pointer", what);
  static unsigned long long lds_ok = 0;
  SPACAP_CHECK_HIP(spacap::allow_dynamic_lds(reinterpret_cast<const void *>(&rel_fused_bwd_kernel), (int)BWD_LDS, lds_ok), what);
  SPACAP_REQUIRE(nparts >= 1 && nparts <= B * (K / TJ) * (K / TI) && zslots >= du_slots(B, K, nparts),
                 "%s: (nparts=%d, zslots=%d) do not fit (B=%d, K=%d)", what, nparts, zslots, B, K);
  hipLaunchKernelGGL(rel_fused_bwd_kernel, dim3(nparts), dim3(256), BWD_LDS, spacap::as_stream(stream), dpred, hid2, P, U, b1, W2, W3, B, K,
                     zslots, dP, dU, part);
  SPACAP_CHECK_LAUNCH(what);
  return SPACAP_OK;
}

static int rel_sel_lists(const char *what, const float *dpred, int B, int K, int zslots, float *dP, float *dU, void *workspace,
                         spacap_stream_t stream) {
  SPACAP_REQUIRE(B >= 0 && K >= 8 && K % 8 == 0 && B <= 65535 && zslots >= 1, "%s: (B=%d, K=%d, zslots=%d) unsupported", what, B, K, zslots);
  if (B == 0) return SPACAP_OK;
  SPACAP_REQUIRE(dpred && dP && dU && workspace, "%s: null pointer", what);
  SPACAP_REQUIRE(((uintptr_t)dpred | (uintptr_t)dP | (uintptr_t)dU) % 16 == 0 && (uintptr_t)workspace % 8 == 0, "%s: unaligned buffer", what);
  hipLaunchKernelGGL(rel_sel_scan_kernel, dim3((unsigned)B * K), dim3(256), 0, spacap::as_stream(stream), dpred, B, K, zslots,
                     static_cast<int *>(workspace), dP, dU);
  SPACAP_CHECK_LAUNCH(what);
  hipLaunchKernelGGL(rel_sel_compact_kernel, dim3(B), dim3(256), 0, spacap::as_stream(stream), B, K, static_cast<int *>(workspace));
  SPACAP_CHECK_LAUNCH(what);
  return SPACAP_OK;
}

extern "C" int spacap_relation_fused_sel_lists_f32(const float *dpred, int B, int K, int zslots, float *dP, float *dU, void *workspace,
                                                   spacap_stream_t stream) {
  return rel_sel_lists("spacap_relation_fused_sel_lists_f32", dpred, B, K, zslots, dP, dU, workspace, stream);
}

extern "C" int spacap_relation_fused_bwd_sel_f32(const float *dpred, const float *hid2, const float *P, const float *U, const float *b1,
                                                 const float *W2, const float *W3, int B, int K, int nparts, int zslots, float *dP,
                                                 float *dU, float *part, void *workspace, spacap_stream_t stream) {
  const char *what = "spacap_relation_fused_bwd_sel_f32";
  SPACAP_REQUIRE(B >= 0 && K >= 8 && K % 8 == 0 && B <= 65535, "%s: (B=%d, K=%d) unsupported", what, B, K);
  if (B == 0) return SPACAP_OK;
  SPACAP_REQUIRE(dpred && hid2 && P && U && b1 && W2 && W3 && dP && dU && part && workspace, "%s: null pointer", what);
  static unsigned long long lds_ok = 0;
  SPACAP_CHECK_HIP(spacap::allow_dynamic_lds(reinterpret_cast<const void *>(&rel_fused_bwd_sel_kernel), (int)BWD_LDS, lds_ok), what);
  SPACAP_REQUIRE(nparts >= 1 && nparts <= B * (K / TJ) * (K / TI) && zslots >= std::max(3, du_slots(B, K, nparts)),
                 "%s: (nparts=%d, zslots=%d) do not fit (B=%d, K=%d)", what, nparts, zslots, B, K);
  if (const int rc = rel_sel_lists(what, dpred, B, K, zslots, dP, dU, workspace, stream)) return rc;
  hipLaunchKernelGGL(rel_fused_bwd_sel_kernel, dim3(nparts), dim3(256), BWD_LDS, spacap::as_stream(stream), dpred, hid2, P, U, b1, W2, W3,
                     B, K, zslots, static_cast<const int *>(workspace), dP, dU, part);
  SPACAP_CHECK_LAUNCH(what);
  return SPACAP_OK;
}
```

spacap3d_amd/relation.py:

```python
import torch
import torch.nn.functional as F
from torch.autograd import Function

from ._native import check, lib, sum_slabs
from .linear import _dense, bf3_pieces, bf3_product, dense_product


class RelationFeature(Function):

    @staticmethod
    def forward(ctx, P, V):
        if not P.is_cuda:
            raise RuntimeError("CPU not supported")
        P = P.contiguous()
        if V.stride(3) != 1 or any(s % 4 for s in V.stride()[:3]) or V.data_ptr() % 16:
            V = V.contiguous()
        B, H, K, D = V.shape
        with torch.cuda.device(P.device):
            R = torch.empty(B, K, K, H * D, dtype=torch.float32, device=P.device)
            check(lib.spacap_relation_feature_fwd_f32(P.data_ptr(), V.data_ptr(), V.stride(0), V.stride(1), V.stride(2),
                                                      B, H, K, D, R.data_ptr(),
                                                      torch.cuda.current_stream(P.device).cuda_stream),
                  "spacap_relation_feature_fwd_f32")
        ctx.save_for_backward(P, V)
        return R

    @staticmethod
    def backward(ctx, dR):
        P, V = ctx.saved_tensors
        B, H, K, D = V.shape
        dR = dR.contiguous()
        with torch.cuda.device(P.device):
            dP = torch.empty_like(P)
            dV = torch.empty(B, K, H, D, dtype=torch.float32, device=P.device)
            check(lib.spacap_relation_feature_bwd_f32(dR.data_ptr(), P.data_ptr(), V.data_ptr(), V.stride(0), V.stride(1),
                                                      V.stride(2), B, H, K, D, dP.data_ptr(), dV.data_ptr(),
                                                      torch.cuda.current_stream(P.device).cuda_stream),
                  "spacap_relation_feature_bwd_f32")
        return dP, dV.transpose(1, 2)


def relation_feature(P, V):
    return RelationFeature.apply(P, V)


class RelationLayer1(Function):

    @staticmethod
    def forward(ctx, P, U, b1):
        P, U = P.contiguous(), U.contiguous()
        B, H, K, _ = P.shape
        C = U.shape[-1]
        with torch.cuda.device(P.device):
            H1 = torch.empty(B, K, K, C, dtype=torch.float32, device=P.device)
            check(lib.spacap_relation_l1_fwd_f32(P.data_ptr(), U.data_ptr(), b1.data_ptr(), B, H, K, C, H1.data_ptr(),
                                                 torch.cuda.current_stream(P.device).cuda_stream), "spacap_relation_l1_fwd_f32")
        ctx.save_for_backward(P, U, H1)
        return H1

    @staticmethod
    def backward(ctx, dH1):
        P, U, H1 = ctx.saved_tensors
        B, H, K, _ = P.shape
        C = U.shape[-1]
        dH1 = dH1.contiguous()
        with torch.cuda.device(P.device):
            dP = torch.empty_like(P)
            dU = torch.empty(int(lib.spacap_relation_l1_isplit()), *U.shape, dtype=torch.float32, device=P.device)
            part = torch.empty(int(lib.spacap_relation_l1_blocks(B, K, C)), C, dtype=torch.float32, device=P.device)
            check(lib.spacap_relation_l1_bwd_f32(dH1.data_ptr(), H1.data_ptr(), P.data_ptr(), U.data_ptr(), B, H, K, C,
                                                 dP.data_ptr(), dU.data_ptr(), part.data_ptr(),
                                                 torch.cuda.current_stream(P.device).cuda_stream), "spacap_relation_l1_bwd_f32")
        return dP, sum_slabs(dU), sum_slabs(part)


def relation_layer1(P, V, weight, bias):
    if not P.is_cuda:
        raise RuntimeError("CPU not supported")
    B, H, K, D = V.shape
    C = weight.shape[0]
    if not lib.spacap_relation_l1_supported(H, K, C):
        return torch.relu(torch.nn.functional.linear(RelationFeature.apply(P, V), weight, bias))
    U = torch.einsum("bhjd,ohd->bjho", V, weight.view(C, H, D))
    return RelationLayer1.apply(P, U, bias)


def _sum_slabs(t):
    if not t.is_cuda:
        return t.sum(0)
    return sum_slabs(t.contiguous())


class _TallLinear(torch.autograd.Function):

    SLABS = 64

    @staticmethod
    def forward(ctx, x, weight, bias):
        ctx.save_for_backward(x, weight)
        return F.linear(x, weight, bias)

    @staticmethod
    def backward(ctx, g):
        x, weight = ctx.saved_tensors
        g2 = g.reshape(-1, g.shape[-1])
        x2 = x.reshape(-1, x.shape[-1])
        rows, S = g2.shape[0], _TallLinear.SLABS
        dx = (g2 @ weight).view_as(x) if ctx.needs_input_grad[0] else None
        if rows % S == 0 and rows >= 64 * S:
            dw = _sum_slabs(torch.bmm(g2.view(S, rows // S, -1).transpose(1, 2), x2.view(S, rows // S, -1)))
        else:
            dw = g2.t() @ x2
        db = g2.view(1024, rows // 1024, -1).sum(1).sum(0) if rows % 1024 == 0 and rows >= 65536 else g2.sum(0)
        return dx, dw, db


def tall_linear(x, lin):
    return _TallLinear.apply(x, lin.weight, lin.bias)


class RelationTail(Function):

    SLABS = 64

    @staticmethod
    def forward(ctx, hid1, W2, b2, W3, b3):
        shape = hid1.shape
        h1 = hid1.reshape(-1, 128).contiguous()
        R = h1.shape[0]
        dev = h1.device
        W2c, W3c = W2.contiguous(), W3.contiguous()
        with torch.cuda.device(dev):
            hid2 = torch.empty_like(h1)
            pred = torch.empty(R, W3.shape[0], dtype=torch.float32, device=dev)
            check(lib.spacap_rel_tail_fwd_f32(h1.data_ptr(), W2c.data_ptr(), b2.data_ptr(), W3c.data_ptr(), b3.data_ptr(), R,
                                              hid2.data_ptr(), pred.data_ptr(), torch.cuda.current_stream(dev).cuda_stream),
                  "spacap_rel_tail_fwd_f32")
        ctx.save_for_backward(h1, hid2, W2c, W3c)
        ctx.shape = shape
        return pred.view(*shape[:-1], W3.shape[0])

    @staticmethod
    def backward(ctx, g):
        h1, hid2, W2, W3 = ctx.saved_tensors
        NO = W3.shape[0]
        g2 = g.reshape(-1, NO).contiguous()
        R = g2.shape[0]
        dev = g2.device
        with torch.cuda.device(dev):
            nparts = int(lib.spacap_rel_tail_bwd_nparts(R))
            PW = NO * 128 + 128 + 16
            part = torch.empty(nparts, PW, dtype=torch.float32, device=dev)
            dz2 = torch.empty_like(hid2)
            check(lib.spacap_rel_tail_bwd_f32(g2.data_ptr(), W3.data_ptr(), hid2.data_ptr(), R, dz2.data_ptr(), part.data_ptr(),
                                              torch.cuda.current_stream(dev).cuda_stream), "spacap_rel_tail_bwd_f32")
            s = sum_slabs(part, deferrable=True)
            dW3, db2, db3 = s[:NO * 128].view(NO, 128), s[NO * 128:NO * 128 + 128], s[NO * 128 + 128:NO * 128 + 128 + NO]
            dh1 = None
            if ctx.needs_input_grad[0]:
                if R >= 49152 and lib.spacap_gemm_rows_supported(128, 128):
                    dh1 = torch.empty_like(hid2)
                    W2t = W2.t().contiguous()
                    check(lib.spacap_gemm_rows_f32(dz2.data_ptr(), W2t.data_ptr(), R, 128, 128, dh1.data_ptr(),
                                                   torch.cuda.current_stream(dev).cuda_stream), "spacap_gemm_rows_f32")
                    dh1 = dh1.view(ctx.shape)
                else:
                    dh1 = (dz2 @ W2).view(ctx.shape)
            S = RelationTail.SLABS
            if R % S == 0 and R >= 64 * S:
                dW2 = sum_slabs(torch.bmm(dz2.view(S, R // S, 128).transpose(1, 2), h1.view(S, R // S, 128)).view(S, -1),
                                deferrable=True).view(128, 128)
            else:
                dW2 = dz2.t() @ h1
        return dh1, dW2, db2, dW3, db3


def relation_tail(hid1, lin2, lin3):
    if not hid1.is_cuda or hid1.dtype != torch.float32 or tuple(lin2.weight.shape) != (128, 128) or \
            tuple(lin3.weight.shape) != (9, 128) or lin2.bias is None or lin3.bias is None or hid1.shape[-1] != 128:
        return None
    return RelationTail.apply(hid1, lin2.weight, lin2.bias, lin3.weight, lin3.bias)


class RelationU(Function):

    @staticmethod
    def forward(ctx, V, W1):
        B, H, K, D = V.shape
        C = W1.shape[0]
        Vr = V.transpose(1, 2)
        if not (Vr.stride(3) == 1 and Vr.stride(2) == D and Vr.stride(0) == K * Vr.stride(1)):
            Vr = Vr.contiguous()
        W1c = W1.contiguous()
        lda = Vr.stride(1)
        dev = V.device
        with torch.cuda.device(dev):
            U = torch.empty(B, K, H, C, dtype=torch.float32, device=dev)
            _dense(dev, Vr.data_ptr(), lda, W1c.data_ptr(), H * D, True, None, B * K, D, C, U.data_ptr(), H * C, slices=H,
                   slice_stride=C, batch=1, a_z=D, w_z=D)
        ctx.save_for_backward(Vr, W1c)
        return U

    @staticmethod
    def backward(ctx, dU):
        Vr, W1 = ctx.saved_tensors
        B, K, H, D = Vr.shape
        C = W1.shape[0]
        R = B * K
        dev = dU.device
        dU = dU.contiguous()
        lda = Vr.stride(1)
        st = torch.cuda.current_stream(dev).cuda_stream
        with torch.cuda.device(dev):
            dV = None
            if ctx.needs_input_grad[0]:
                dVr = torch.empty(B, K, H, D, dtype=torch.float32, device=dev)
                _dense(dev, dU.data_ptr(), H * C, W1.data_ptr(), H * D, False, None, R, C, D, dVr.data_ptr(), H * D, slices=H,
                       slice_stride=D, batch=1, a_z=C, w_z=D)
                dV = dVr.transpose(1, 2)
            nslab = int(lib.spacap_dense_wgrad_blocks_slabs(R))
            part = torch.empty(nslab, C * H * D, dtype=torch.float32, device=dev)
            check(lib.spacap_dense_wgrad_blocks_f32(dU.data_ptr(), H * C, Vr.data_ptr(), lda, R, H, C, D, nslab, part.data_ptr(), st),
                  "spacap_dense_wgrad_blocks_f32")
            dW1 = sum_slabs(part, deferrable=True).view(C, H * D)
        return dV, dW1


class RelationHead(Function):

    @staticmethod
    def forward(ctx, P, U, b1, W2, b2, W3, b3):
        P, U, W2c, W3c = P.contiguous(), U.contiguous(), W2.contiguous(), W3.contiguous()
        B, H, K, _ = P.shape
        dev = P.device
        with torch.cuda.device(dev):
            hid2 = torch.empty(B, K, K, 128, dtype=torch.float32, device=dev)
            pred = torch.empty(B, K, K, 9, dtype=torch.float32, device=dev)
            check(lib.spacap_relation_fused_fwd_f32(P.data_ptr(), U.data_ptr(), b1.data_ptr(), W2c.data_ptr(), b2.data_ptr(),
                                                    W3c.data_ptr(), b3.data_ptr(), B, K, hid2.data_ptr(), pred.data_ptr(),
                                                    torch.cuda.current_stream(dev).cuda_stream), "spacap_relation_fused_fwd_f32")
        ctx.save_for_backward(P, U, b1, W2c, W3c, hid2)
        return pred

    @staticmethod
    def backward(ctx, g):
        P, U, b1, W2, W3, hid2 = ctx.saved_tensors
        B, H, K, _ = P.shape
        dev = P.device
        g = g.contiguous()
        with torch.cuda.device(dev):
            PW = int(lib.spacap_relation_fused_part_floats())
            nparts = int(lib.spacap_relation_fused_nparts(B, K))
            zslots = int(lib.spacap_relation_fused_sel_zsplit(B, K, nparts))
            part = torch.empty(nparts, PW, dtype=torch.float32, device=dev)
            dP = torch.empty_like(P)
            dU = torch.empty(zslots, *U.shape, dtype=torch.float32, device=dev)
            ws = torch.empty(int(lib.spacap_relation_fused_sel_workspace_bytes(B, K)), dtype=torch.uint8, device=dev)
            check(lib.spacap_relation_fused_bwd_sel_f32(g.data_ptr(), hid2.data_ptr(), P.data_ptr(), U.data_ptr(), b1.data_ptr(),
                                                        W2.data_ptr(), W3.data_ptr(), B, K, nparts, zslots, dP.data_ptr(),
                                                        dU.data_ptr(), part.data_ptr(), ws.data_ptr(),
                                                        torch.cuda.current_stream(dev).cuda_stream),
                  "spacap_relation_fused_bwd_sel_f32")
            s = sum_slabs(part, deferrable=True)
        o = 128 * 128
        dW2, dW3 = s[:o].view(128, 128), s[o:o + 9 * 128].view(9, 128)
        o += 9 * 128
        return dP, sum_slabs(dU), s[o:o + 128], dW2, s[o + 128:o + 256], dW3, s[o + 256:o + 265]


class RelationWide(Function):

    @staticmethod
    def forward(ctx, P, U, b1, W2, b2, W3, b3):
        P, U, W2c, W3c = P.contiguous(), U.contiguous(), W2.contiguous(), W3.contiguous()
        B, H, K, _ = P.shape
        C = U.shape[-1]
        dev = P.device
        st = torch.cuda.current_stream(dev).cuda_stream
        with torch.cuda.device(dev):
            Pt = torch.empty(B, K, H, K, dtype=torch.float32, device=dev)
            check(lib.spacap_rel_wide_transpose_f32(P.data_ptr(), Pt.data_ptr(), B, H, K, 1, st), "spacap_rel_wide_transpose_f32")
            hid1 = torch.empty(B * K * K, C, dtype=torch.float32, device=dev)
            check(lib.spacap_rel_wide_l1_fwd_f32(Pt.data_ptr(), U.data_ptr(), b1.data_ptr(), B, H, K, C, hid1.data_ptr(), st),
                  "spacap_rel_wide_l1_fwd_f32")
            hid2 = bf3_product(hid1, bf3_pieces(W2c), b2, relu=True)
            pred = dense_product(hid2, W3c, True, bias=b3)
        ctx.save_for_backward(Pt, U, W2c, W3c, hid1, hid2)
        ctx.spent = False
        return pred.view(B, K, K, W3c.shape[0])

    @staticmethod
    def backward(ctx, g):
        if ctx.spent:
            raise RuntimeError("RelationWide: its backward can run once per forward (retain_graph is not supported)")
        ctx.spent = True
        Pt, U, W2, W3, hid1, hid2 = ctx.saved_tensors
        B, K, H, _ = Pt.shape
        C = U.shape[-1]
        NO = W3.shape[0]
        R = B * K * K
        dev = Pt.device
        st = torch.cuda.current_stream(dev).cuda_stream
        g2 = g.reshape(R, NO).contiguous()
        with torch.cuda.device(dev):
            nparts = int(lib.spacap_rel_wide_tail_nparts(R))
            part = torch.empty(nparts, NO * C + C + 16, dtype=torch.float32, device=dev)
            dz2 = torch.empty_like(hid2)
            check(lib.spacap_rel_wide_tail_bwd_f32(g2.data_ptr(), W3.data_ptr(), hid2.data_ptr(), R, C, nparts, dz2.data_ptr(),
                                                   part.data_ptr(), st), "spacap_rel_wide_tail_bwd_f32")
            s = sum_slabs(part, deferrable=True)
            dW3, db2, db3 = s[:NO * C].view(NO, C), s[NO * C:NO * C + C], s[NO * C + C:NO * C + C + NO]
            nslab = int(lib.spacap_gemm_bf3_wgrad_slabs(R, C, C))
            pw = torch.empty(nslab, C * C, dtype=torch.float32, device=dev)
            check(lib.spacap_linear_wgrad_nslab_f32(dz2.data_ptr(), hid1.data_ptr(), R, C, C, 0, nslab, pw.data_ptr(), st),
                  "spacap_linear_wgrad_nslab_f32")
            dW2 = sum_slabs(pw, deferrable=True).view(C, C)
            dh1 = bf3_product(dz2, bf3_pieces(W2, trans=True), out=hid2)
            del dz2
            dPt, dU = torch.empty_like(Pt), torch.empty_like(U)
            pb = torch.empty(B * K, C, dtype=torch.float32, device=dev)
            check(lib.spacap_rel_wide_l1_bwd_f32(dh1.data_ptr(), hid1.data_ptr(), Pt.data_ptr(), U.data_ptr(), B, H, K, C, dPt.data_ptr(),
                                                 dU.data_ptr(), pb.data_ptr(), st), "spacap_rel_wide_l1_bwd_f32")
            dP = torch.empty(B, H, K, K, dtype=torch.float32, device=dev)
            check(lib.spacap_rel_wide_transpose_f32(dPt.data_ptr(), dP.data_ptr(), B, H, K, 0, st), "spacap_rel_wide_transpose_f32")
        return dP, dU, sum_slabs(pb), dW2, db2, dW3, db3



def _fused_shape(H, K, C, NO):
    return C == 128 and bool(lib.spacap_relation_fused_supported(H, K, 128, NO))


def _wide_shape(H, K, C, NO):
    return NO == 9 and bool(lib.spacap_rel_wide_l1_supported(H, K, C)) and bool(lib.spacap_gemm_bf3_supported(C, C)) and \
        bool(lib.spacap_rel_wide_tail_supported(C))


def tier(H, K, D, C, NO, cuda, grad):
    if not cuda:
        return None
    if _fused_shape(H, K, C, NO):
        return "fused"
    if _wide_shape(H, K, C, NO):
        return "wide"
    first = "l1" if lib.spacap_relation_l1_supported(H, K, C) else "feature"
    return first + ("+tail" if grad and C == 128 and NO == 9 else "+tall")


def _mlp_of(P, V, lin1, lin2, lin3):
    B, H, K, D = V.shape
    C, NO = lin1.weight.shape[0], lin3.weight.shape[0]
    if not P.is_cuda or P.dtype != torch.float32 or lin1.bias is None or lin2.bias is None or lin3.bias is None or \
            tuple(lin1.weight.shape) != (C, H * D) or tuple(lin2.weight.shape) != (C, C) or lin3.weight.shape[1] != C:
        return None
    return H, K, C, NO


def relation_head_wide(P, V, lin1, lin2, lin3):
    s = _mlp_of(P, V, lin1, lin2, lin3)
    if s is None or not _wide_shape(*s):
        return None
    U = RelationU.apply(V, lin1.weight)
    return RelationWide.apply(P, U, lin1.bias, lin2.weight, lin2.bias, lin3.weight, lin3.bias)


def relation_head(P, V, lin1, lin2, lin3):
    s = _mlp_of(P, V, lin1, lin2, lin3)
    if s is None or not _fused_shape(*s):
        return relation_head_wide(P, V, lin1, lin2, lin3)
    U = RelationU.apply(V, lin1.weight)
    return RelationHead.apply(P, U, lin1.bias, lin2.weight, lin2.bias, lin3.weight, lin3.bias)


def relation_pred(P, V, lin1, lin2, lin3):
    if not P.is_cuda:
        raise RuntimeError("CPU not supported")
    B, H, K, D = V.shape
    t = tier(H, K, D, lin1.weight.shape[0], lin3.weight.shape[0], True, torch.is_grad_enabled())
    pred = None
    if t == "fused":
        pred = relation_head(P, V, lin1, lin2, lin3)
    elif t == "wide":
        pred = relation_head_wide(P, V, lin1, lin2, lin3)
    if pred is None:
        hid = relation_layer1(P, V, lin1.weight, lin1.bias)
        if t.endswith("+tail"):
            pred = relation_tail(hid, lin2, lin3)
        if pred is None:
            pred = tall_linear(F.relu(tall_linear(hid, lin2)), lin3)
    return pred
```

Before: 1205 scenes/s.

## Recompute relation hid2 in backward only for selected tiles instead of storing it

The relation head forward no longer writes the full B×K×K×128 hid2 activation. It only produces predictions. The backward pass adds a recompute kernel that rebuilds hid2 into scratch for just the tiles the selection lists mark as having nonzero gradient, then runs the existing selective backward kernel. This trades a large forward write and its saved-tensor memory for extra layer-1/2 compute in backward, limited to selected tiles. Tile-walking logic is factored into a shared TileWalk helper.

```diff
diff --git a/include/spacap_hip.h b/include/spacap_hip.h
--- a/include/spacap_hip.h
+++ b/include/spacap_hip.h
@@ -130,6 +130,7 @@
                                int K, int C, float *dP, float *dU, float *db_part, spacap_stream_t stream);
 
 int spacap_relation_fused_leave_cus(int n);
+int spacap_relation_fused_fwd_leave_cus(int n);
 int spacap_relation_fused_supported(int H, int K, int C, int n_out);
 int spacap_relation_fused_nparts(int B, int K);
 int spacap_relation_fused_zsplit(int B, int K, int nparts);
@@ -137,6 +138,8 @@
 int spacap_relation_fused_fwd_f32(const float *P, const float *U, const float *b1, const float *W2, const float *b2,
                                   const float *W3, const float *b3, int B, int K, float *hid2, float *pred,
                                   spacap_stream_t stream);
+int spacap_relation_fused_fwd_pred_f32(const float *P, const float *U, const float *b1, const float *W2, const float *b2,
+                                       const float *W3, const float *b3, int B, int K, float *pred, spacap_stream_t stream);
 int spacap_relation_fused_bwd_f32(const float *dpred, const float *hid2, const float *P, const float *U, const float *b1,
                                   const float *W2, const float *W3, int B, int K, int nparts, int zslots, float *dP,
                                   float *dU, float *part, spacap_stream_t stream);
@@ -147,6 +150,9 @@
 int spacap_relation_fused_bwd_sel_f32(const float *dpred, const float *hid2, const float *P, const float *U, const float *b1,
                                       const float *W2, const float *W3, int B, int K, int nparts, int zslots, float *dP,
                                       float *dU, float *part, void *workspace, spacap_stream_t stream);
+int spacap_relation_fused_bwd_sel_rc_f32(const float *dpred, const float *P, const float *U, const float *b1, const float *W2,
+                                         const float *b2, const float *W3, int B, int K, int nparts, int zslots, float *dP,
+                                         float *dU, float *part, void *workspace, float *hid2_scratch, spacap_stream_t stream);
 
 int spacap_caption_prep_fwd_f32(const float *xyz, const float *ref, const float *src, const float *memory,
                                 const int64_t *tok, const float *emb, const float *pe, int B, int K, int D, int T, int V,
diff --git a/spacap3d_amd/_native.py b/spacap3d_amd/_native.py
--- a/spacap3d_amd/_native.py
+++ b/spacap3d_amd/_native.py
@@ -62,6 +62,9 @@
     "spacap_relation_fused_sel_workspace_bytes": (ctypes.c_size_t, [_i, _i]),
     "spacap_relation_fused_sel_lists_f32": (_i, [_p, _i, _i, _i, _p, _p, _p, _p]),
     "spacap_relation_fused_bwd_sel_f32": (_i, [_p] * 7 + [_i, _i, _i, _i, _p, _p, _p, _p, _p]),
+    "spacap_relation_fused_fwd_leave_cus": (_i, [_i]),
+    "spacap_relation_fused_fwd_pred_f32": (_i, [_p] * 7 + [_i, _i, _p, _p]),
+    "spacap_relation_fused_bwd_sel_rc_f32": (_i, [_p] * 7 + [_i, _i, _i, _i, _p, _p, _p, _p, _p, _p]),
     "spacap_caption_prep_fwd_f32": (_i, [_p] * 7 + [_i] * 5 + [_f, _u64, _p] + [_p] * 7 + [_p]),
     "spacap_caption_prep_bwd_f32": (_i, [_p] * 3 + [_i] * 5 + [_f, _u64, _p, _p, _p, _p]),
     "spacap_caption_prep_rows_fwd_f32": (_i, [_p] * 6 + [_i] * 7 + [_f, _u64, _p] + [_p] * 2 + [_p]),
diff --git a/spacap3d_amd/csrc/relation_fused.hip b/spacap3d_amd/csrc/relation_fused.hip
--- a/spacap3d_amd/csrc/relation_fused.hip
+++ b/spacap3d_amd/csrc/relation_fused.hip
@@ -76,6 +76,52 @@
   }
 }
 
+template <bool PRED>
+__device__ __forceinline__ void fwd_weights(const float *__restrict__ W2, const float *__restrict__ b2, const float *__restrict__ W3,
+                                            int w, int l15, int lg, bf16x8 (&wA)[2][4][3], float (&w3r)[2][4], f32x4 (&bb)[2]) {
+#pragma unroll
+  for (int t = 0; t < 2; ++t) {
+    const float *wp = W2 + (size_t)(32 * w + 16 * t + l15) * C + 8 * lg;
+#pragma unroll
+    for (int kc = 0; kc < 4; ++kc) split8(ld4(wp + 32 * kc), ld4(wp + 32 * kc + 4), wA[t][kc]);
+#pragma unroll
+    for (int uu = 0; uu < 4; ++uu) w3r[t][uu] = PRED && l15 < NO ? W3[l15 * C + 32 * w + 16 * t + 4 * lg + uu] : 0.f;
+    bb[t] = ld4(b2 + 32 * w + 16 * t + 4 * lg);
+  }
+}
+
+template <bool STORE, bool PRED, class PairOf>
+__device__ __forceinline__ void fwd_layers23(const __bf16 *s_a, const bf16x8 (&wA)[2][4][3], const float (&w3r)[2][4], const f32x4 (&bb)[2],
+                                             int w, int l15, int lg, float *__restrict__ hid2, float *s_pr, PairOf pair_of) {
+#pragma unroll 2
+  for (int mt = 0; mt < TR / 16; ++mt) {
+    f32x4 acc[2] = {{0.f, 0.f, 0.f, 0.f}, {0.f, 0.f, 0.f, 0.f}};
+#pragma unroll
+    for (int kc = 0; kc < 4; ++kc) {
+      bf16x8 a[3];
+      ld_pieces(s_a + (mt * 16 + l15) * LDB + 32 * kc + 8 * lg, IMG, a);
+      acc[0] = mfma6(wA[0][kc], a, acc[0]);
+      acc[1] = mfma6(wA[1][kc], a, acc[1]);
+    }
+    const int rr = mt * 16 + l15;
+    float *hrow = STORE ? hid2 + pair_of(rr) * C + 32 * w + 4 * lg : nullptr;
+    f32x4 a3 = {0.f, 0.f, 0.f, 0.f}, a3b = {0.f, 0.f, 0.f, 0.f};
+#pragma unroll
+    for (int t = 0; t < 2; ++t) {
+      const f32x4 h = relu4(acc[t] + bb[t]);
+      if (STORE) st4(hrow + 16 * t, h);
+      if (PRED) {
+        a3 = MFMA16(w3r[t][0], h[0], a3);
+        a3b = MFMA16(w3r[t][1], h[1], a3b);
+        a3 = MFMA16(w3r[t][2], h[2], a3);
+        a3b = MFMA16(w3r[t][3], h[3], a3b);
+      }
+    }
+    if (PRED && lg < 3) st4(&s_pr[(w * TR + rr) * DPL + 4 * lg], a3 + a3b);
+  }
+}
+
+template <bool STORE_H2>
 __global__ __launch_bounds__(256) void rel_fused_fwd_kernel(const float *__restrict__ P, const float *__restrict__ Um,
                                                             const float *__restrict__ b1, const float *__restrict__ W2,
                                                             const float *__restrict__ b2, const float *__restrict__ W3,
@@ -91,15 +137,7 @@
   bf16x8 wA[2][4][3];
   float w3r[2][4];
   f32x4 bb[2];
-#pragma unroll
-  for (int t = 0; t < 2; ++t) {
-    const float *wp = W2 + (size_t)(32 * w + 16 * t + l15) * C + 8 * lg;
-#pragma unroll
-    for (int kc = 0; kc < 4; ++kc) split8(ld4(wp + 32 * kc), ld4(wp + 32 * kc + 4), wA[t][kc]);
-#pragma unroll
-    for (int uu = 0; uu < 4; ++uu) w3r[t][uu] = l15 < NO ? W3[l15 * C + 32 * w + 16 * t + 4 * lg + uu] : 0.f;
-    bb[t] = ld4(b2 + 32 * w + 16 * t + 4 * lg);
-  }
+  fwd_weights<true>(W2, b2, W3, w, l15, lg, wA, w3r, bb);
   float pp[2];
   for (long u = u_beg; u < u_end;) {
     const int grp = (int)(u / NI), ib0 = (int)(u - (long)grp * NI), ibe = (int)min((long)NI, ib0 + (u_end - u));
@@ -132,30 +170,7 @@
       __syncthreads();
       hid1_rows<false>(uA, bA, s_p, w, l15, lg, s_a);
       __syncthreads();
-#pragma unroll 2
-      for (int mt = 0; mt < TR / 16; ++mt) {
-        f32x4 acc[2] = {{0.f, 0.f, 0.f, 0.f}, {0.f, 0.f, 0.f, 0.f}};
-#pragma unroll
-        for (int kc = 0; kc < 4; ++kc) {
-          bf16x8 a[3];
-          ld_pieces(s_a + (mt * 16 + l15) * LDB + 32 * kc + 8 * lg, IMG, a);
-          acc[0] = mfma6(wA[0][kc], a, acc[0]);
-          acc[1] = mfma6(wA[1][kc], a, acc[1]);
-        }
-        const int rr = mt * 16 + l15;
-        float *hrow = hid2 + pair_row(b, K, i0, j0, rr) * C + 32 * w + 4 * lg;
-        f32x4 a3 = {0.f, 0.f, 0.f, 0.f}, a3b = {0.f, 0.f, 0.f, 0.f};
-#pragma unroll
-        for (int t = 0; t < 2; ++t) {
-          const f32x4 h = relu4(acc[t] + bb[t]);
-          st4(hrow + 16 * t, h);
-          a3 = MFMA16(w3r[t][0], h[0], a3);
-          a3b = MFMA16(w3r[t][1], h[1], a3b);
-          a3 = MFMA16(w3r[t][2], h[2], a3);
-          a3b = MFMA16(w3r[t][3], h[3], a3b);
-        }
-        if (lg < 3) st4(&s_pr[(w * TR + rr) * DPL + 4 * lg], a3 + a3b);
-      }
+      fwd_layers23<STORE_H2, true>(s_a, wA, w3r, bb, w, l15, lg, hid2, s_pr, [&](int rr) { return pair_row(b, K, i0, j0, rr); });
     }
     __syncthreads();
     pred_out(iend - TI);
@@ -172,6 +187,88 @@
 __host__ __device__ inline size_t sel_blk_off(int B, int K) { return sel_colbits_off(B, K) + (size_t)2 * B * K * sel_nw(K); }
 __host__ __device__ inline int sel_blk_stride(int K) { return 2 + 2 * (K / 8); }
 __device__ __forceinline__ int clampi(int v, int hi) { return min(max(v, 0), hi); }
+
+template <bool SEL>
+struct TileWalk {
+  int B, K, NI, NJ, BS;
+  const int *ws, *cnt, *blk;
+  long NU, u_beg, u_end, L;
+  bool dense;
+  int sc, NIs, NJs;
+  long sbeg;
+  int b, j0, ib0, ibe;
+  long kstart;
+  const int *rfl, *ql, *kl;
+
+  __device__ __forceinline__ void init(const int *ws_, int B_, int K_, int Z, void *scratch) {
+    const int tid = threadIdx.x, lane = tid & 63, w = tid >> 6;
+    ws = ws_, B = B_, K = K_, NI = K / TI, NJ = K / TJ;
+    NU = (long)B * NJ * NI, u_beg = (long)blockIdx.x * NU / gridDim.x, u_end = ((long)blockIdx.x + 1) * NU / gridDim.x;
+    L = 0, dense = true;
+    cnt = SEL ? ws + sel_cnt_off(B, K) : nullptr, blk = SEL ? ws + sel_blk_off(B, K) : nullptr;
+    BS = sel_blk_stride(K);
+    if (SEL) {
+      long long nu = 0, tb = 0;
+      int nim = 0;
+      for (int s = tid; s < B; s += 256) {
+        const int ni = clampi(cnt[4 * s + 2], NI), nj = clampi(cnt[4 * s + 3], NJ);
+        nu += (long long)ni * nj;
+        nim = max(nim, ni);
+        tb += (long long)clampi(blk[(size_t)s * BS], NI) * clampi(blk[(size_t)s * BS + 1], NJ);
+      }
+#pragma unroll
+      for (int m = 32; m >= 1; m >>= 1) {
+        nu += __shfl_xor(nu, m);
+        tb += __shfl_xor(tb, m);
+        nim = max(nim, __shfl_xor(nim, m));
+      }
+      long long *s_nu = reinterpret_cast<long long *>(scratch);
+      int *s_ni = reinterpret_cast<int *>(s_nu + 8);
+      if (lane == 0) s_nu[w] = nu, s_nu[4 + w] = tb, s_ni[w] = nim;
+      __syncthreads();
+      nu = (s_nu[0] + s_nu[1]) + (s_nu[2] + s_nu[3]);
+      tb = (s_nu[4] + s_nu[5]) + (s_nu[6] + s_nu[7]);
+      nim = max(max(s_ni[0], s_ni[1]), max(s_ni[2], s_ni[3]));
+      dense = tb <= nu || tb * 16 <= NU;
+      if (!dense) {
+        NU = nu;
+        L = max((NU + gridDim.x - 1) / gridDim.x, (long)(nim + max(Z - 1, 1) - 1) / max(Z - 1, 1));
+        u_beg = min(NU, (long)blockIdx.x * L);
+        u_end = min(NU, ((long)blockIdx.x + 1) * L);
+      }
+    }
+    sc = 0, sbeg = 0, NIs = NI, NJs = NJ;
+    if (SEL && u_beg < u_end) NIs = clampi(cnt[2], NI), NJs = clampi(cnt[3], NJ);
+    b = j0 = ib0 = ibe = 0, kstart = 0, rfl = ql = kl = nullptr;
+  }
+  __device__ __forceinline__ void stretch(long &u) {
+    if (SEL && !dense) {
+      while (sc + 1 < B && u >= sbeg + (long)NIs * NJs) {
+        sbeg += (long)NIs * NJs;
+        ++sc;
+        NIs = clampi(cnt[4 * sc + 2], NI), NJs = clampi(cnt[4 * sc + 3], NJ);
+      }
+      const long v = u - sbeg;
+      const int jb = (int)(v / NIs);
+      ib0 = (int)(v - (long)jb * NIs), ibe = (int)min((long)NIs, ib0 + (u_end - u));
+      b = sc, j0 = jb * TJ, kstart = sbeg + (long)jb * NIs;
+    } else {
+      const int grp = (int)(u / NI);
+      ib0 = (int)(u - (long)grp * NI), ibe = (int)min((long)NI, ib0 + (u_end - u));
+      b = grp / NJ, j0 = (grp - b * NJ) * TJ, kstart = (long)grp * NI;
+    }
+    u += ibe - ib0;
+    if (SEL) rfl = blk + (size_t)b * BS + 2, ql = ws + sel_qi_off(B, K) + (size_t)b * K, kl = ws + sel_kj_off(B, K) + (size_t)b * K;
+  }
+  __device__ __forceinline__ bool key_block_idle() const { return SEL && dense && !rfl[NI + (j0 >> 3)]; }
+  __device__ __forceinline__ int next_tile(int ib) const {
+    if (SEL && dense)
+      while (ib < ibe && !rfl[ib]) ++ib;
+    return ib;
+  }
+  __device__ __forceinline__ int key(int x) const { return SEL && !dense ? clampi(kl[j0 + x], K - 1) : j0 + x; }
+  __device__ __forceinline__ int query(int i0, int x) const { return SEL && !dense ? clampi(ql[i0 + x], K - 1) : i0 + x; }
+};
 
 template <bool SEL>
 __device__ __forceinline__ void rel_bwd_body(const float *__restrict__ dpred, const float *__restrict__ hid2,
@@ -187,46 +284,15 @@
   float *s_p = s_x + TR * LDT, *s_dp = s_p + H * TR;
   const int tid = threadIdx.x, lane = tid & 63, w = tid >> 6, l15 = lane & 15, lg = lane >> 4;
   const int jj = tid >> 5, c4 = tid & 31;
-  const int NI = K / TI, NJ = K / TJ;
-  long NU = (long)B * NJ * NI, u_beg = (long)blockIdx.x * NU / gridDim.x, u_end = ((long)blockIdx.x + 1) * NU / gridDim.x;
-  long L = 0;
-  bool dense = true;
-  const int *cnt = SEL ? ws + sel_cnt_off(B, K) : nullptr, *blk = SEL ? ws + sel_blk_off(B, K) : nullptr;
-  const int BS = sel_blk_stride(K);
-  if (SEL) {
-    long long nu = 0, tb = 0;
-    int nim = 0;
-    for (int s = tid; s < B; s += 256) {
-      const int ni = clampi(cnt[4 * s + 2], NI), nj = clampi(cnt[4 * s + 3], NJ);
-      nu += (long long)ni * nj;
-      nim = max(nim, ni);
-      tb += (long long)clampi(blk[(size_t)s * BS], NI) * clampi(blk[(size_t)s * BS + 1], NJ);
-    }
-#pragma unroll
-    for (int m = 32; m >= 1; m >>= 1) {
-      nu += __shfl_xor(nu, m);
-      tb += __shfl_xor(tb, m);
-      nim = max(nim, __shfl_xor(nim, m));
-    }
-    long long *s_nu = reinterpret_cast<long long *>(s_x);
-    int *s_ni = reinterpret_cast<int *>(s_nu + 8);
-    if (lane == 0) s_nu[w] = nu, s_nu[4 + w] = tb, s_ni[w] = nim;
-    __syncthreads();
-    nu = (s_nu[0] + s_nu[1]) + (s_nu[2] + s_nu[3]);
-    tb = (s_nu[4] + s_nu[5]) + (s_nu[6] + s_nu[7]);
-    nim = max(max(s_ni[0], s_ni[1]), max(s_ni[2], s_ni[3]));
-    dense = tb <= nu || tb * 16 <= NU;
-    if (!dense) {
-      NU = nu;
-      L = max((NU + gridDim.x - 1) / gridDim.x, (long)(nim + max(Z - 1, 1) - 1) / max(Z - 1, 1));
-      u_beg = min(NU, (long)blockIdx.x * L);
-      u_end = min(NU, ((long)blockIdx.x + 1) * L);
-    }
-    if (u_beg >= u_end) {
-      float *po = part + (size_t)blockIdx.x * PART;
-      for (int idx = tid; idx < PART; idx += 256) po[idx] = 0.f;
-      return;
-    }
+  TileWalk<SEL> wk;
+  wk.init(ws, B, K, Z, s_x);
+  const int NI = wk.NI;
+  const long NU = wk.NU, L = wk.L;
+  const bool dense = wk.dense;
+  if (SEL && wk.u_beg >= wk.u_end) {
+    float *po = part + (size_t)blockIdx.x * PART;
+    for (int idx = tid; idx < PART; idx += 256) po[idx] = 0.f;
+    return;
   }
   float bA[8], w3A[8][3];
 #pragma unroll
@@ -255,39 +321,16 @@
 
   f32x4 hp[TI];
   float pp[2], dq[3];
-  int sc = 0, NIs = SEL ? clampi(cnt[2], NI) : NI, NJs = SEL ? clampi(cnt[3], NJ) : NJ;
-  long sbeg = 0;
-  for (long u = u_beg; u < u_end;) {
-  int b, j0, ib0, ibe;
-  long kstart;
-  if (SEL && !dense) {
-    while (sc + 1 < B && u >= sbeg + (long)NIs * NJs) {
-      sbeg += (long)NIs * NJs;
-      ++sc;
-      NIs = clampi(cnt[4 * sc + 2], NI), NJs = clampi(cnt[4 * sc + 3], NJ);
-    }
-    const long v = u - sbeg;
-    const int jb = (int)(v / NIs);
-    ib0 = (int)(v - (long)jb * NIs), ibe = (int)min((long)NIs, ib0 + (u_end - u));
-    b = sc, j0 = jb * TJ, kstart = sbeg + (long)jb * NIs;
-  } else {
-    const int grp = (int)(u / NI);
-    ib0 = (int)(u - (long)grp * NI), ibe = (int)min((long)NI, ib0 + (u_end - u));
-    b = grp / NJ, j0 = (grp - b * NJ) * TJ, kstart = (long)grp * NI;
-  }
-  u += ibe - ib0;
-  const int *rfl = SEL ? blk + (size_t)b * BS + 2 : nullptr;
-  auto next_tile = [&](int ib) -> int {
-    if (SEL && dense)
-      while (ib < ibe && !rfl[ib]) ++ib;
-    return ib;
-  };
-  if (SEL && dense && !rfl[NI + (j0 >> 3)]) continue;
+  for (long u = wk.u_beg; u < wk.u_end;) {
+  wk.stretch(u);
+  const int b = wk.b, ib0 = wk.ib0, ibe = wk.ibe;
+  const long kstart = wk.kstart;
+  auto next_tile = [&](int ib) -> int { return wk.next_tile(ib); };
+  if (wk.key_block_idle()) continue;
   int ib = next_tile(ib0);
   if (ib >= ibe) continue;
   int ibn = next_tile(ib + 1), ibn2 = ibn < ibe ? next_tile(ibn + 1) : ibe;
-  const int *ql = SEL ? ws + sel_qi_off(B, K) + (size_t)b * K : nullptr, *kl = SEL ? ws + sel_kj_off(B, K) + (size_t)b * K : nullptr;
-  auto KJ = [&](int x) -> int { return SEL && !dense ? clampi(kl[j0 + x], K - 1) : j0 + x; };
+  auto KJ = [&](int x) -> int { return wk.key(x); };
   const int kP = KJ(tid & 7), kH = KJ(jj), kU[2] = {KJ(2 * w), KJ(2 * w + 1)}, kR = KJ(2 * w + (l15 >> 3)), kZ = KJ(2 * w + (lg >> 1));
   int kD[3], iD[3], oD[3];
 #pragma unroll
@@ -305,7 +348,7 @@
     du[n] = f32x4{0.f, 0.f, 0.f, 0.f};
   }
   int ha = 0, hb = 0;
-  auto rows_of = [&](int i0) -> int { return !SEL ? 0 : dense ? i0 + (lane & 7) : clampi(ql[i0 + (lane & 7)], K - 1); };
+  auto rows_of = [&](int i0) -> int { return !SEL ? 0 : wk.query(i0, lane & 7); };
   auto row = [&](int i0, int h, int x) -> int { return SEL ? __shfl(h, x & 7) : i0 + x; };
   auto request = [&](int i0, int h) {
     p_tile_request_at(P, b, K, row(i0, h, (tid >> 3) & 7), kP, pp);
@@ -509,6 +552,51 @@
                                                                 const int *__restrict__ ws, float *__restrict__ dP,
                                                                 float *__restrict__ dU, float *__restrict__ part) {
   rel_bwd_body<true>(dpred, hid2, P, U, b1, W2, W3, B, K, Z, ws, dP, dU, part);
+}
+
+__global__ __launch_bounds__(256) void rel_fused_rc_kernel(const float *__restrict__ P, const float *__restrict__ Um,
+                                                           const float *__restrict__ b1, const float *__restrict__ W2,
+                                                           const float *__restrict__ b2, int B, int K, int Z,
+                                                           const int *__restrict__ ws, float *__restrict__ hid2) {
+  extern __shared__ __attribute__((aligned(16))) unsigned char smem_raw[];
+  __bf16 *s_a = reinterpret_cast<__bf16 *>(smem_raw);
+  float *s_p = reinterpret_cast<float *>(smem_raw + 3 * IMG * 2);
+  const int tid = threadIdx.x, lane = tid & 63, w = tid >> 6, l15 = lane & 15, lg = lane >> 4;
+  TileWalk<true> wk;
+  wk.init(ws, B, K, Z, s_p);
+  if (wk.u_beg >= wk.u_end) return;
+  bf16x8 wA[2][4][3];
+  float w3r[2][4];
+  f32x4 bb[2];
+  fwd_weights<false>(W2, b2, nullptr, w, l15, lg, wA, w3r, bb);
+  float pp[2];
+  for (long u = wk.u_beg; u < wk.u_end;) {
+    wk.stretch(u);
+    if (wk.key_block_idle()) continue;
+    int ib = wk.next_tile(wk.ib0);
+    if (ib >= wk.ibe) continue;
+    const int b = wk.b, kP = wk.key(tid & 7), kU[2] = {wk.key(2 * w), wk.key(2 * w + 1)};
+    float uA[8][4], bA[8];
+#pragma unroll
+    for (int n = 0; n < 8; ++n) {
+#pragma unroll
+      for (int ks = 0; ks < 4; ++ks) uA[n][ks] = Um[(((size_t)b * K + kU[ks >> 1]) * H + 4 * (ks & 1) + lg) * C + 16 * n + l15];
+      bA[n] = lg == 0 ? b1[16 * n + l15] : 0.f;
+    }
+    p_tile_request_at(P, b, K, wk.query(ib * TI, (tid >> 3) & 7), kP, pp);
+    while (ib < wk.ibe) {
+      const int i0 = ib * TI, ibn = wk.next_tile(ib + 1);
+      const size_t qS = ((size_t)b * K + wk.query(i0, l15 & 7)) * K;
+      __syncthreads();
+      p_tile_store(pp, s_p);
+      if (ibn < wk.ibe) p_tile_request_at(P, b, K, wk.query(ibn * TI, (tid >> 3) & 7), kP, pp);
+      __syncthreads();
+      hid1_rows<false>(uA, bA, s_p, w, l15, lg, s_a);
+      __syncthreads();
+      fwd_layers23<true, false>(s_a, wA, w3r, bb, w, l15, lg, hid2, nullptr, [&](int rr) { return qS + wk.key(2 * (rr >> 4) + (l15 >> 3)); });
+      ib = ibn;
+    }
+  }
 }
 
 __global__ __launch_bounds__(256) void rel_sel_scan_kernel(const float *__restrict__ dpred, int B, int K, int Z, int *__restrict__ ws,
@@ -609,11 +697,13 @@
 
 constexpr size_t FWD_LDS = (size_t)3 * IMG * 2 + (size_t)(4 * TR * DPL + H * TR) * sizeof(float);
 constexpr size_t BWD_LDS = (size_t)2 * 3 * IMGT * 2 + (size_t)(TR * LDT + H * TR + TR * DPL) * sizeof(float);
-
-static std::atomic<int> g_rel_leave{0};
-inline int grid_size(int B, int K, int per_cu) {
+constexpr size_t RC_LDS = (size_t)3 * IMG * 2 + (size_t)(H * TR) * sizeof(float);
+
+static std::atomic<int> g_rel_leave{0}, g_rel_fwd_leave{-1};
+inline int grid_size(int B, int K, int per_cu, bool fwd = false) {
   const long units = (long)B * (K / TJ) * (K / TI);
-  const int extra = g_rel_leave.load(std::memory_order_relaxed);
+  int extra = g_rel_leave.load(std::memory_order_relaxed);
+  if (fwd && g_rel_fwd_leave.load(std::memory_order_relaxed) >= 0) extra = g_rel_fwd_leave.load(std::memory_order_relaxed);
   const long g = (long)per_cu * std::max(1, spacap::device_cus() - extra - spacap::launch::fwd_cus_left_free(per_cu));
   return (int)std::min(units, g);
 }
@@ -634,6 +724,11 @@
   g_rel_leave.store(n, std::memory_order_relaxed);
   return SPACAP_OK;
 }
+extern "C" int spacap_relation_fused_fwd_leave_cus(int n) {
+  if (n < -1 || n > spacap::device_cus() * 3 / 4) return SPACAP_E_INVALID;
+  g_rel_fwd_leave.store(n, std::memory_order_relaxed);
+  return SPACAP_OK;
+}
 extern "C" int spacap_relation_fused_supported(int H_, int K, int C_, int NO_) {
   return H_ == H && C_ == C && NO_ == NO && K >= 8 && K % 8 == 0;
 }
@@ -647,19 +742,28 @@
   return B > 0 && K >= 8 ? (sel_blk_off(B, K) + (size_t)B * sel_blk_stride(K)) * sizeof(int) : 0;
 }
 
+template <bool STORE_H2>
+static int rel_fwd(const char *what, const float *P, const float *U, const float *b1, const float *W2, const float *b2, const float *W3,
+                   const float *b3, int B, int K, float *hid2, float *pred, spacap_stream_t stream) {
+  SPACAP_REQUIRE(B >= 0 && K >= 8 && K % 8 == 0 && B <= 65535, "%s: (B=%d, K=%d) unsupported", what, B, K);
+  if (B == 0) return SPACAP_OK;
+  SPACAP_REQUIRE(P && U && b1 && W2 && b2 && W3 && b3 && (hid2 || !STORE_H2) && pred, "%s: null pointer", what);
+  static unsigned long long lds_ok = 0;
+  SPACAP_CHECK_HIP(spacap::allow_dynamic_lds(reinterpret_cast<const void *>(&rel_fused_fwd_kernel<STORE_H2>), (int)FWD_LDS, lds_ok), what);
+  hipLaunchKernelGGL(rel_fused_fwd_kernel<STORE_H2>, dim3(grid_size(B, K, 2, true)), dim3(256), FWD_LDS, spacap::as_stream(stream), P, U,
+                     b1, W2, b2, W3, b3, B, K, hid2, pred);
+  SPACAP_CHECK_LAUNCH(what);
+  return SPACAP_OK;
+}
+
 extern "C" int spacap_relation_fused_fwd_f32(const float *P, const float *U, const float *b1, const float *W2, const float *b2,
                                              const float *W3, const float *b3, int B, int K, float *hid2, float *pred,
                                              spacap_stream_t stream) {
-  const char *what = "spacap_relation_fused_fwd_f32";
-  SPACAP_REQUIRE(B >= 0 && K >= 8 && K % 8 == 0 && B <= 65535, "%s: (B=%d, K=%d) unsupported", what, B, K);
-  if (B == 0) return SPACAP_OK;
-  SPACAP_REQUIRE(P && U && b1 && W2 && b2 && W3 && b3 && hid2 && pred, "%s: null pointer", what);
-  static unsigned long long lds_ok = 0;
-  SPACAP_CHECK_HIP(spacap::allow_dynamic_lds(reinterpret_cast<const void *>(&rel_fused_fwd_kernel), (int)FWD_LDS, lds_ok), what);
-  hipLaunchKernelGGL(rel_fused_fwd_kernel, dim3(grid_size(B, K, 2)), dim3(256), FWD_LDS, spacap::as_stream(stream), P, U, b1, W2, b2, W3,
-                     b3, B, K, hid2, pred);
-  SPACAP_CHECK_LAUNCH(what);
-  return SPACAP_OK;
+  return rel_fwd<true>("spacap_relation_fused_fwd_f32", P, U, b1, W2, b2, W3, b3, B, K, hid2, pred, stream);
+}
+extern "C" int spacap_relation_fused_fwd_pred_f32(const float *P, const float *U, const float *b1, const float *W2, const float *b2,
+                                                  const float *W3, const float *b3, int B, int K, float *pred, spacap_stream_t stream) {
+  return rel_fwd<false>("spacap_relation_fused_fwd_pred_f32", P, U, b1, W2, b2, W3, b3, B, K, nullptr, pred, stream);
 }
 
 extern "C" int spacap_relation_fused_bwd_f32(const float *dpred, const float *hid2, const float *P, const float *U, const float *b1,
@@ -698,20 +802,43 @@
   return rel_sel_lists("spacap_relation_fused_sel_lists_f32", dpred, B, K, zslots, dP, dU, workspace, stream);
 }
 
-extern "C" int spacap_relation_fused_bwd_sel_f32(const float *dpred, const float *hid2, const float *P, const float *U, const float *b1,
-                                                 const float *W2, const float *W3, int B, int K, int nparts, int zslots, float *dP,
-                                                 float *dU, float *part, void *workspace, spacap_stream_t stream) {
-  const char *what = "spacap_relation_fused_bwd_sel_f32";
+static int rel_bwd_sel(const char *what, const float *dpred, float *hid2, const float *P, const float *U, const float *b1, const float *W2,
+                       const float *b2, const float *W3, int B, int K, int nparts, int zslots, float *dP, float *dU, float *part,
+                       void *workspace, spacap_stream_t stream) {
   SPACAP_REQUIRE(B >= 0 && K >= 8 && K % 8 == 0 && B <= 65535, "%s: (B=%d, K=%d) unsupported", what, B, K);
   if (B == 0) return SPACAP_OK;
   SPACAP_REQUIRE(dpred && hid2 && P && U && b1 && W2 && W3 && dP && dU && part && workspace, "%s: null pointer", what);
-  static unsigned long long lds_ok = 0;
+  static unsigned long long lds_ok = 0, rc_lds_ok = 0;
   SPACAP_CHECK_HIP(spacap::allow_dynamic_lds(reinterpret_cast<const void *>(&rel_fused_bwd_sel_kernel), (int)BWD_LDS, lds_ok), what);
+  if (b2) {
+    SPACAP_CHECK_HIP(spacap::allow_dynamic_lds(reinterpret_cast<const void *>(&rel_fused_rc_kernel), (int)RC_LDS, rc_lds_ok), what);
+  }
   SPACAP_REQUIRE(nparts >= 1 && nparts <= B * (K / TJ) * (K / TI) && zslots >= std::max(3, du_slots(B, K, nparts)),
                  "%s: (nparts=%d, zslots=%d) do not fit (B=%d, K=%d)", what, nparts, zslots, B, K);
   if (const int rc = rel_sel_lists(what, dpred, B, K, zslots, dP, dU, workspace, stream)) return rc;
+  if (b2) {
+    SPACAP_REQUIRE((uintptr_t)hid2 % 16 == 0, "%s: unaligned buffer", what);
+    hipLaunchKernelGGL(rel_fused_rc_kernel, dim3(nparts), dim3(256), RC_LDS, spacap::as_stream(stream), P, U, b1, W2, b2, B, K, zslots,
+                       static_cast<const int *>(workspace), hid2);
+    SPACAP_CHECK_LAUNCH(what);
+  }
   hipLaunchKernelGGL(rel_fused_bwd_sel_kernel, dim3(nparts), dim3(256), BWD_LDS, spacap::as_stream(stream), dpred, hid2, P, U, b1, W2, W3,
                      B, K, zslots, static_cast<const int *>(workspace), dP, dU, part);
   SPACAP_CHECK_LAUNCH(what);
   return SPACAP_OK;
 }
+
+extern "C" int spacap_relation_fused_bwd_sel_f32(const float *dpred, const float *hid2, const float *P, const float *U, const float *b1,
+                                                 const float *W2, const float *W3, int B, int K, int nparts, int zslots, float *dP,
+                                                 float *dU, float *part, void *workspace, spacap_stream_t stream) {
+  return rel_bwd_sel("spacap_relation_fused_bwd_sel_f32", dpred, const_cast<float *>(hid2), P, U, b1, W2, nullptr, W3, B, K, nparts, zslots,
+                     dP, dU, part, workspace, stream);
+}
+extern "C" int spacap_relation_fused_bwd_sel_rc_f32(const float *dpred, const float *P, const float *U, const float *b1, const float *W2,
+                                                    const float *b2, const float *W3, int B, int K, int nparts, int zslots, float *dP,
+                                                    float *dU, float *part, void *workspace, float *hid2_scratch,
+                                                    spacap_stream_t stream) {
+  const char *what = "spacap_relation_fused_bwd_sel_rc_f32";
+  SPACAP_REQUIRE(b2 || B == 0, "%s: null pointer", what);
+  return rel_bwd_sel(what, dpred, hid2_scratch, P, U, b1, W2, b2, W3, B, K, nparts, zslots, dP, dU, part, workspace, stream);
+}
diff --git a/spacap3d_amd/relation.py b/spacap3d_amd/relation.py
--- a/spacap3d_amd/relation.py
+++ b/spacap3d_amd/relation.py
@@ -228,26 +228,37 @@
 
 class RelationHead(Function):
 
+    STORE_HID2 = False
+
     @staticmethod
     def forward(ctx, P, U, b1, W2, b2, W3, b3):
         P, U, W2c, W3c = P.contiguous(), U.contiguous(), W2.contiguous(), W3.contiguous()
         B, H, K, _ = P.shape
         dev = P.device
-        with torch.cuda.device(dev):
-            hid2 = torch.empty(B, K, K, 128, dtype=torch.float32, device=dev)
+        st = torch.cuda.current_stream(dev).cuda_stream
+        with torch.cuda.device(dev):
             pred = torch.empty(B, K, K, 9, dtype=torch.float32, device=dev)
-            check(lib.spacap_relation_fused_fwd_f32(P.data_ptr(), U.data_ptr(), b1.data_ptr(), W2c.data_ptr(), b2.data_ptr(),
-                                                    W3c.data_ptr(), b3.data_ptr(), B, K, hid2.data_ptr(), pred.data_ptr(),
-                                                    torch.cuda.current_stream(dev).cuda_stream), "spacap_relation_fused_fwd_f32")
-        ctx.save_for_backward(P, U, b1, W2c, W3c, hid2)
+            if RelationHead.STORE_HID2:
+                hid2 = torch.empty(B, K, K, 128, dtype=torch.float32, device=dev)
+                check(lib.spacap_relation_fused_fwd_f32(P.data_ptr(), U.data_ptr(), b1.data_ptr(), W2c.data_ptr(), b2.data_ptr(),
+                                                        W3c.data_ptr(), b3.data_ptr(), B, K, hid2.data_ptr(), pred.data_ptr(), st),
+                      "spacap_relation_fused_fwd_f32")
+                ctx.save_for_backward(P, U, b1, W2c, W3c, hid2)
+            else:
+                check(lib.spacap_relation_fused_fwd_pred_f32(P.data_ptr(), U.data_ptr(), b1.data_ptr(), W2c.data_ptr(), b2.data_ptr(),
+                                                             W3c.data_ptr(), b3.data_ptr(), B, K, pred.data_ptr(), st),
+                      "spacap_relation_fused_fwd_pred_f32")
+                ctx.save_for_backward(P, U, b1, W2c, W3c, b2)
+        ctx.stored = RelationHead.STORE_HID2
         return pred
 
     @staticmethod
     def backward(ctx, g):
-        P, U, b1, W2, W3, hid2 = ctx.saved_tensors
+        P, U, b1, W2, W3, last = ctx.saved_tensors
         B, H, K, _ = P.shape
         dev = P.device
         g = g.contiguous()
+        st = torch.cuda.current_stream(dev).cuda_stream
         with torch.cuda.device(dev):
             PW = int(lib.spacap_relation_fused_part_floats())
             nparts = int(lib.spacap_relation_fused_nparts(B, K))
@@ -256,11 +267,17 @@
             dP = torch.empty_like(P)
             dU = torch.empty(zslots, *U.shape, dtype=torch.float32, device=dev)
             ws = torch.empty(int(lib.spacap_relation_fused_sel_workspace_bytes(B, K)), dtype=torch.uint8, device=dev)
-            check(lib.spacap_relation_fused_bwd_sel_f32(g.data_ptr(), hid2.data_ptr(), P.data_ptr(), U.data_ptr(), b1.data_ptr(),
-                                                        W2.data_ptr(), W3.data_ptr(), B, K, nparts, zslots, dP.data_ptr(),
-                                                        dU.data_ptr(), part.data_ptr(), ws.data_ptr(),
-                                                        torch.cuda.current_stream(dev).cuda_stream),
-                  "spacap_relation_fused_bwd_sel_f32")
+            if ctx.stored:
+                check(lib.spacap_relation_fused_bwd_sel_f32(g.data_ptr(), last.data_ptr(), P.data_ptr(), U.data_ptr(), b1.data_ptr(),
+                                                            W2.data_ptr(), W3.data_ptr(), B, K, nparts, zslots, dP.data_ptr(),
+                                                            dU.data_ptr(), part.data_ptr(), ws.data_ptr(), st),
+                      "spacap_relation_fused_bwd_sel_f32")
+            else:
+                scratch = torch.empty(B, K, K, 128, dtype=torch.float32, device=dev)
+                check(lib.spacap_relation_fused_bwd_sel_rc_f32(g.data_ptr(), P.data_ptr(), U.data_ptr(), b1.data_ptr(), W2.data_ptr(),
+                                                               last.data_ptr(), W3.data_ptr(), B, K, nparts, zslots, dP.data_ptr(),
+                                                               dU.data_ptr(), part.data_ptr(), ws.data_ptr(), scratch.data_ptr(), st),
+                      "spacap_relation_fused_bwd_sel_rc_f32")
             s = sum_slabs(part, deferrable=True)
         o = 128 * 128
         dW2, dW3 = s[:o].view(128, 128), s[o:o + 9 * 128].view(9, 128)
```

Result: no change. 1212 scenes/s (median of 6 runs) (+0.6%).
